# highfem/tqdne

Measured on AMD Instinct MI355X. Metric: waveforms/sec (train step + 18-step EDM sample), 3ch x 4096, higher is better.
Workload: dtype f32 (contractions on MFMA with fp32 accumulate: bf16x3, and fp16 + block-scaled-fp6 corrections on the 128/256-channel forward convs; sampler state f64)

## Files before the change

include/tqdne_hip.h:

```cpp
#ifndef TQDNE_HIP_H
#define TQDNE_HIP_H

#include <stddef.h>
#include <stdint.h>

#ifdef __cplusplus
extern "C" {
#endif

#ifndef __HIP__
typedef struct ihipStream_t* hipStream_t;
#endif

#define TQ_ABI_VERSION 8

#define TQ_ERR_ARG (-1)
#define TQ_ERR_SHAPE (-2)

#define TQ_CONV_GN 1
#define TQ_CONV_SILU 2
#define TQ_CONV_EMB 4
#define TQ_CONV_RES 8
#define TQ_CONV_STATS 16
#define TQ_CONV_DROPOUT 32
#define TQ_CONV_POLY2 64
#define TQ_CONV_CH_TILES 128
#define TQ_CONV_WIDE_TABLE 256

#define TQ_WFMT_BF16X3 0
#define TQ_WFMT_F16_MX8 1
#define TQ_WFMT_F16_MX6 2

typedef struct TqGnFold {
    const float* stats0;
    const float* stats1;
    int32_t slot0, slot1;
    const float* gamma;
    const float* beta;
    float* mean_rstd;
} TqGnFold;

typedef struct TqConvDesc {
    int32_t B, T_in, T_out;
    int32_t C_in0, C_in1;
    int32_t C_out;
    int32_t ktaps, stride, pad;
    int32_t upsample;
    int32_t flags;
    int32_t emb_stride;
    uint32_t dropout_site;
    float dropout_p;
    uint64_t dropout_seed;
    int32_t C_skip0, C_skip1;
    int32_t wfmt;
    int32_t* range_flag;
    const void* reserved1;
    int32_t t_tile;
    int32_t reserved2;
    const TqGnFold* gn_fold;
} TqConvDesc;

#define TQ_BWD_GN 1
#define TQ_BWD_SILU 2
#define TQ_BWD_DROPOUT 4
#define TQ_BWD_ACCUM 8
#define TQ_BWD_STATS 16

typedef struct TqConvBwdDesc {
    int32_t B, T;
    int32_t C_dy;
    int32_t C_dx0, C_dx1;
    int32_t ktaps;
    int32_t flags;
    uint32_t dropout_site;
    float dropout_p;
    uint64_t dropout_seed;
    int32_t wfmt;
    int32_t reserved;
    const uint32_t* dy_amax;
} TqConvBwdDesc;

int tq_abi_version(void);
int tq_build_flags(void);

size_t tq_conv_weight_pack_bytes(int C_out, int C_in, int K, int mode);
int tq_pack_conv_weight(const float* w, int C_out, int C_in, int K, int mode, void* packed, hipStream_t stream);
int tq_conv_tile_co(int C_out);
int tq_conv1d_max_cin(int wfmt, int C_out);
int tq_conv1d_max_cout(void);
size_t tq_conv1d_wide_lds_bytes(int ktaps, int t_tile, int C_out);
int tq_conv1d_gn_table_entries(int wide);
int tq_conv1d_gn_fold_max_cin(int wfmt, int t_tile, int C_out);
int tq_colsum_max_channels(void);
typedef struct TqPackJob {
    const void* src;
    void* dst;
    int32_t C_out, C_in, K, mode;
    int32_t block_begin;
    int32_t reserved;
} TqPackJob;
int tq_pack_job_blocks(int C_out, int C_in, int K, int mode);
int tq_pack_jobs(const TqPackJob* jobs_device, int njobs, int total_blocks, hipStream_t stream);

int tq_conv1d_fwd(const TqConvDesc* desc, const float* x0, const float* x1, const float* gscale, const float* gshift,
                  const void* packed_w, const float* bias, const float* emb, const float* residual, float* y,
                  float* stats_partial, hipStream_t stream);

int tq_conv1d_fwd_skip(const TqConvDesc* desc, const float* x0, const float* x1, const float* gscale, const float* gshift,
                       const void* packed_w_main_then_skip, const float* bias, const float* emb, const float* skip_x0,
                       const float* skip_x1, const float* skip_bias, float* y, float* stats_partial, hipStream_t stream);

#define TQ_KV_V_BF16 0
#define TQ_KV_V_F16 1
int tq_conv1d_fwd_qkv(const TqConvDesc* desc, const float* x, const float* gscale, const float* gshift, const void* packed_w,
                      const float* bias, float* qkv, void* kv_planes, int H, int D, int v_format, hipStream_t stream);

int tq_conv1d_bwd_data(const TqConvBwdDesc* desc, const float* dy, const void* packed_w_t, const float* x0, const float* x1,
                       const float* gscale, const float* gshift, float* dx0, float* dx1, float* gstats_partial,
                       hipStream_t stream);

size_t tq_conv1d_bwd_weight_workspace(const TqConvDesc* desc);
int tq_conv1d_bwd_weight(const TqConvDesc* desc, const float* dy, const float* x0, const float* x1, const float* gscale,
                         const float* gshift, float* dw, void* workspace, size_t ws_bytes, hipStream_t stream);
int tq_conv1d_bwd_weight_colsum(const TqConvDesc* desc, const float* dy, const float* x0, const float* x1, const float* gscale,
                                const float* gshift, float* dw, void* workspace, size_t ws_bytes, float* colsum_bc, int bc_stride,
                                float* colsum_c, float* colsum_c2, hipStream_t stream);

size_t tq_stem_conv_lds_bytes(int C_in, int C_out, int ktaps);
int tq_stem_conv_fwd(const float* x_nct, const float* in_scale, const float* w, const float* bias, float* y,
                     float* stats_partial, int B, int C_in, int T, int C_out, int ktaps, hipStream_t stream);

size_t tq_head_conv_lds_bytes(int C_in, int C_out, int ktaps);
int tq_head_conv_fwd(const float* x, const float* gscale, const float* gshift, const float* w, const float* bias,
                     const float* c_out, const float* c_skip, const float* skip_src, float* y_nct, int B, int T, int C_in,
                     int C_out, int ktaps, hipStream_t stream);

int tq_gn_finalize(const float* stats0, int C0, const float* stats1, int C1, int B, int T, const float* gamma,
                   const float* beta, float* gscale, float* gshift, float* mean_rstd, int slot0, int slot1, hipStream_t stream);

int tq_gn_bwd_finalize(const float* gstats_partial, const float* mean_rstd, const float* gamma, int B, int C, int T,
                       float* coef_a, float* coef_b, float* coef_c, float* dgamma, float* dbeta, hipStream_t stream);
int tq_gn_bwd_apply(const float* g, const float* x, const float* r, const float* coef_a, const float* coef_b,
                    const float* coef_c, float* dx, int B, int T, int C_src, int C_total, int c_offset, int accumulate,
                    hipStream_t stream);
int tq_gn_bwd_apply_colsum(const float* g, const float* x, const float* r, const float* coef_a, const float* coef_b,
                           const float* coef_c, float* dx, int B, int T, int C_src, int C_total, int c_offset, int accumulate,
                           float* colsum_bc, int bc_stride, float* colsum_c, float* colsum_c2, uint32_t* amax_out,
                           hipStream_t stream);
typedef struct TqGemmJob {
    const float* A;
    const float* B;
    float* C;
    const float* U;
    int32_t M, N, K;
    int32_t sam, sak, sbk, sbn, ldc, ldu;
    int32_t pre_b;
    int32_t tile_begin;
} TqGemmJob;
int tq_gemm_tiles(int M, int N);
int tq_gemm_f32_jobs(const TqGemmJob* jobs_device, int njobs, int total_tiles, hipStream_t stream);
int tq_fourier_features(const float* t, const float* W, float* out, int B, int half, hipStream_t stream);

#define TQ_AMAX_WAYS 16
#define TQ_AMAX_STRIDE 32
#define TQ_AMAX_WORDS (TQ_AMAX_WAYS * TQ_AMAX_STRIDE)
int tq_colsum(const float* dy, int B, int T, int C, float* out_bc, int bc_stride, float* out_c, float* out_c2,
              const float* bscale, uint32_t* amax_out, hipStream_t stream);
int tq_zero_stuff(const float* dy, float* out, int B, int T_out, int T_in, int C, hipStream_t stream);
int tq_pair_sum(const float* d_up, float* dx, int B, int T, int C, int accumulate, hipStream_t stream);
int tq_upsample_poly_wgrad_fold(const float* dw2, float* dw, int C_out, int C_in, hipStream_t stream);
int tq_stem_conv_bwd_weight(const float* dy, const float* x_nct, const float* in_scale, float* dw, int B, int C_in, int T,
                            int C_out, int ktaps, hipStream_t stream);
size_t tq_stem_head_bwd_workspace(void);
int tq_stem_conv_bwd_weight_ws(const float* dy, const float* x_nct, const float* in_scale, float* dw, int B, int C_in, int T,
                               int C_out, int ktaps, void* workspace, size_t ws_bytes, hipStream_t stream);
int tq_head_conv_bwd_ws(const float* dpred_nct, const float* c_out, const float* x, const float* gscale, const float* gshift,
                        const float* w, float* g_out, float* gstats_partial, float* dw, float* db, int B, int T, int C_in,
                        int C_out, int ktaps, void* workspace, size_t ws_bytes, hipStream_t stream);
size_t tq_head_conv_bwd_lds_bytes(int C_in, int C_out, int ktaps);
int tq_head_conv_bwd(const float* dpred_nct, const float* c_out, const float* x, const float* gscale, const float* gshift,
                     const float* w, float* g_out, float* gstats_partial, float* dw, float* db, int B, int T, int C_in,
                     int C_out, int ktaps, hipStream_t stream);

int tq_embed_fwd(const float* t, const float* cond, const float* fourier_w, const float* w0, const float* b0,
                 const float* w2, const float* b2, const float* cw0, const float* cb0, const float* cw2, const float* cb2,
                 float* emb, float* silu_emb, float* hidden ,
                 int B, int mc, int ncond, hipStream_t stream);

int tq_linear_fwd(const float* x, const float* w, const float* bias, float* out, int B, int E, int N, hipStream_t stream);

size_t tq_attention_workspace_bytes(int B, int T, int H, int D);
int tq_attention_fwd(const float* qkv, float* out, float* lse ,
                     void* workspace , int B, int T,
                     int H, int D, hipStream_t stream);
int tq_attention_fwd_presplit(const float* qkv, const void* kv_planes, float* out, int B, int T, int H, int D, int v_format,
                              hipStream_t stream);
int tq_attention_bwd(const float* qkv, const float* out, const float* dout, const float* lse, float* delta, float* dqkv, int B,
                     int T, int H, int D, hipStream_t stream);
int tq_attention_bwd_ws(const float* qkv, const float* out, const float* dout, const float* lse, float* delta, float* dqkv,
                        void* workspace, int B, int T, int H, int D, hipStream_t stream);
int tq_attention_bwd_ws_kv(const float* qkv, const float* out, const float* dout, const float* lse, float* delta, float* dqkv,
                           void* workspace, const void* kv_planes, int B, int T, int H, int D, hipStream_t stream);

int tq_attention_head_tile(int D);
size_t tq_attention_hd_lds_bytes(int D, int pass);
size_t tq_attention_hd_workspace_bytes(int B, int T, int H, int D);
int tq_attention_fwd_hd(const float* qkv, float* out, float* lse, void* workspace, int B, int T, int H, int D, hipStream_t stream);
int tq_attention_bwd_hd(const float* qkv, const float* out, const float* dout, const float* lse, float* delta, float* dqkv,
                        void* workspace, int B, int T, int H, int D, hipStream_t stream);

int tq_edm_scalars(const float* sigma, int sigma_stride, float sigma_data, float* c_in, float* c_out, float* c_skip,
                   float* c_noise, float* lweight, int B, hipStream_t stream);
int tq_cm_scalars(const float* sigma, int sigma_stride, float sigma_data, float sigma_min, float* c_out, float* c_skip,
                  int B, hipStream_t stream);
int tq_edm_noise_inject(const float* y, const float* unit_noise, const float* eps, float P_mean, float P_std,
                        float* sigma, float* x_noisy, int B, int n_per_sample, hipStream_t stream);
int tq_edm_loss(const float* pred, const float* y, const float* lweight, float* loss_out, float* dpred, int B,
                int n_per_sample, hipStream_t stream);
// ... 90 lines not shown
```

tqdne_amd/_lib.py:

```python

from __future__ import annotations

import ctypes as C
import os
from typing import Optional

from . import _build

_LIB = None

c_f32p = C.c_void_p
VP = C.c_void_p
I = C.c_int
F = C.c_float
SZ = C.c_size_t

TQ_CONV_GN, TQ_CONV_SILU, TQ_CONV_EMB, TQ_CONV_RES, TQ_CONV_STATS, TQ_CONV_DROPOUT = 1, 2, 4, 8, 16, 32
TQ_CONV_POLY2 = 64
TQ_CONV_CH_TILES = 128
TQ_CONV_WIDE_TABLE = 256
TQ_WFMT_BF16X3, TQ_WFMT_F16_MX8, TQ_WFMT_F16_MX6 = 0, 1, 2
TQ_KV_V_BF16, TQ_KV_V_F16 = 0, 1
PACK_MODE = {TQ_WFMT_BF16X3: 0, TQ_WFMT_F16_MX8: 2, TQ_WFMT_F16_MX6: 3}
PACK_MODE_T = {TQ_WFMT_BF16X3: 1, TQ_WFMT_F16_MX6: 5}


DEFAULT_SCHEME = "f16mx6"
ABI_VERSION = 8


def requested_scheme() -> str:
    v = os.environ.get("TQDNE_CONV_SCHEME", DEFAULT_SCHEME).lower()
    if v not in ("bf16x3", "f16mx8", "f16mx6"):
        raise ValueError(f"TQDNE_CONV_SCHEME={v!r}: expected bf16x3, f16mx8 or f16mx6")
    return v


def attn_v_format() -> int:
    if os.environ.get("TQDNE_ATTN_VF16", "1") == "0" or requested_scheme() == "bf16x3":
        return TQ_KV_V_BF16
    return TQ_KV_V_F16


MX6_C64 = os.environ.get("TQDNE_CONV_MX6_C64", "0") == "1"


WIDE_MX6 = os.environ.get("TQDNE_WIDE_MX6", "1") != "0"


def conv_max_cin(wfmt: int, C_out: int = 0) -> int:
    return load().tq_conv1d_max_cin(wfmt, C_out)


def forward_wfmt(C_out: int, sources, stride: int = 1, upsample: bool = False, k5_act: bool = False,
                 gn: Optional[bool] = None) -> int:
    v = requested_scheme()
    co_ok = C_out % 128 == 0 or (C_out % 64 == 0 and k5_act and not upsample and v == "f16mx6" and MX6_C64)
    ok = stride == 1 and co_ok and all(c % 64 == 0 for c in sources if c)
    if not ok or v == "bf16x3":
        return TQ_WFMT_BF16X3
    fmt = TQ_WFMT_F16_MX6 if v == "f16mx6" else TQ_WFMT_F16_MX8
    cin = sum(c for c in list(sources)[:2] if c)
    if gn is None or gn:
        if cin > conv_max_cin(fmt, C_out) or (cin > load().tq_conv1d_gn_table_entries(0) and not WIDE_MX6):
            return TQ_WFMT_BF16X3
    return fmt
TQ_BWD_GN, TQ_BWD_SILU, TQ_BWD_DROPOUT, TQ_BWD_ACCUM, TQ_BWD_STATS = 1, 2, 4, 8, 16
STAT_SLOT = 128
TQ_AMAX_WAYS, TQ_AMAX_STRIDE = 16, 32
TQ_AMAX_WORDS = TQ_AMAX_WAYS * TQ_AMAX_STRIDE


class TqGnFold(C.Structure):
    _fields_ = [("stats0", C.c_void_p), ("stats1", C.c_void_p), ("slot0", C.c_int32), ("slot1", C.c_int32),
                ("gamma", C.c_void_p), ("beta", C.c_void_p), ("mean_rstd", C.c_void_p)]


class TqConvDesc(C.Structure):
    _fields_ = [
        ("B", C.c_int32), ("T_in", C.c_int32), ("T_out", C.c_int32),
        ("C_in0", C.c_int32), ("C_in1", C.c_int32), ("C_out", C.c_int32),
        ("ktaps", C.c_int32), ("stride", C.c_int32), ("pad", C.c_int32),
        ("upsample", C.c_int32), ("flags", C.c_int32), ("emb_stride", C.c_int32),
        ("dropout_site", C.c_uint32), ("dropout_p", C.c_float), ("dropout_seed", C.c_uint64),
        ("C_skip0", C.c_int32), ("C_skip1", C.c_int32), ("wfmt", C.c_int32),
        ("range_flag", C.c_void_p), ("reserved1", C.c_void_p), ("t_tile", C.c_int32), ("reserved2", C.c_int32),
        ("gn_fold", C.POINTER(TqGnFold)),
    ]


class TqAdamChunk(C.Structure):
    _fields_ = [("p", C.c_void_p), ("g", C.c_void_p), ("m", C.c_void_p), ("v", C.c_void_p), ("ema", C.c_void_p),
                ("n", C.c_int32), ("reserved", C.c_int32)]


TQ_ADAM_CHUNK = 4096


class TqGemmJob(C.Structure):
    _fields_ = [("A", C.c_void_p), ("B", C.c_void_p), ("C", C.c_void_p), ("U", C.c_void_p),
                ("M", C.c_int32), ("N", C.c_int32), ("K", C.c_int32),
                ("sam", C.c_int32), ("sak", C.c_int32), ("sbk", C.c_int32), ("sbn", C.c_int32), ("ldc", C.c_int32), ("ldu", C.c_int32),
                ("pre_b", C.c_int32), ("tile_begin", C.c_int32)]


class TqPackJob(C.Structure):
    _fields_ = [("src", C.c_void_p), ("dst", C.c_void_p), ("C_out", C.c_int32), ("C_in", C.c_int32), ("K", C.c_int32),
                ("mode", C.c_int32), ("block_begin", C.c_int32), ("reserved", C.c_int32)]


class TqConvBwdDesc(C.Structure):
    _fields_ = [
        ("B", C.c_int32), ("T", C.c_int32), ("C_dy", C.c_int32), ("C_dx0", C.c_int32), ("C_dx1", C.c_int32),
        ("ktaps", C.c_int32), ("flags", C.c_int32), ("dropout_site", C.c_uint32), ("dropout_p", C.c_float),
        ("dropout_seed", C.c_uint64), ("wfmt", C.c_int32), ("reserved", C.c_int32), ("dy_amax", C.c_void_p),
    ]


_PROTOS = {
    "tq_abi_version": (I, []),
    "tq_build_flags": (I, []),
    "tq_conv_weight_pack_bytes": (SZ, [I, I, I, I]),
    "tq_pack_conv_weight": (I, [VP, I, I, I, I, VP, VP]),
    "tq_conv_tile_co": (I, [I]),
    "tq_conv1d_max_cin": (I, [I, I]),
    "tq_conv1d_max_cout": (I, []),
    "tq_conv1d_gn_table_entries": (I, [I]),
    "tq_conv1d_wide_lds_bytes": (SZ, [I, I, I]),
    "tq_conv1d_gn_fold_max_cin": (I, [I, I, I]),
    "tq_colsum_max_channels": (I, []),
    "tq_conv1d_fwd": (I, [C.POINTER(TqConvDesc)] + [VP] * 11),
    "tq_conv1d_fwd_skip": (I, [C.POINTER(TqConvDesc)] + [VP] * 13),
    "tq_stem_conv_fwd": (I, [VP] * 6 + [I] * 5 + [VP]),
    "tq_head_conv_fwd": (I, [VP] * 9 + [I] * 5 + [VP]),
    "tq_head_conv_lds_bytes": (SZ, [I, I, I]),
    "tq_stem_conv_lds_bytes": (SZ, [I, I, I]),
    "tq_head_conv_bwd_lds_bytes": (SZ, [I, I, I]),
    "tq_gn_finalize": (I, [VP, I, VP, I, I, I, VP, VP, VP, VP, VP, I, I, VP]),
    "tq_embed_fwd": (I, [VP] * 14 + [I, I, I, VP]),
    "tq_linear_fwd": (I, [VP] * 4 + [I, I, I, VP]),
    "tq_attention_fwd": (I, [VP, VP, VP, VP, I, I, I, I, VP]),
    "tq_attention_fwd_presplit": (I, [VP, VP, VP, I, I, I, I, I, VP]),
    "tq_conv1d_fwd_qkv": (I, [C.POINTER(TqConvDesc)] + [VP] * 7 + [I, I, I, VP]),
    "tq_attention_workspace_bytes": (SZ, [I, I, I, I]),
    "tq_attention_bwd": (I, [VP] * 6 + [I, I, I, I, VP]),
    "tq_attention_bwd_ws": (I, [VP] * 7 + [I, I, I, I, VP]),
    "tq_attention_bwd_ws_kv": (I, [VP] * 8 + [I, I, I, I, VP]),
    "tq_attention_head_tile": (I, [I]),
    "tq_attention_hd_lds_bytes": (SZ, [I, I]),
    "tq_attention_hd_workspace_bytes": (SZ, [I, I, I, I]),
    "tq_attention_fwd_hd": (I, [VP, VP, VP, VP, I, I, I, I, VP]),
    "tq_attention_bwd_hd": (I, [VP] * 7 + [I, I, I, I, VP]),
    "tq_edm_scalars": (I, [VP, I, F, VP, VP, VP, VP, VP, I, VP]),
    "tq_cm_scalars": (I, [VP, I, F, F, VP, VP, I, VP]),
    "tq_edm_noise_inject": (I, [VP, VP, VP, F, F, VP, VP, I, I, VP]),
    "tq_edm_loss": (I, [VP, VP, VP, VP, VP, I, I, VP]),
    "tq_heun_euler": (I, [VP] * 7 + [SZ, VP]),
    "tq_heun_correct": (I, [VP] * 8 + [SZ, VP]),
    "tq_sampler_init": (I, [VP] * 4 + [SZ, VP]),
    "tq_heun_churn": (I, [VP, VP, VP, C.c_double, VP, VP, SZ, VP]),
    "tq_axpy_sigma": (I, [VP, VP, VP, VP, I, I, VP]),
    "tq_pseudo_huber_loss": (I, [VP, VP, VP, F, VP, VP, I, I, VP]),
    "tq_mse_loss": (I, [VP, VP, VP, VP, SZ, VP]),
    "tq_scale_add2": (I, [VP, VP, VP, VP, VP, I, I, VP]),
    "tq_ddpm_step": (I, [VP, VP, VP, VP, SZ, I] + [C.c_double] * 6 + [VP]),
    "tq_vae_reparam_fwd": (I, [VP, VP, VP, VP, I, I, I, VP]),
    "tq_vae_reparam_bwd": (I, [VP, VP, VP, VP, F, I, I, I, VP]),
    "tq_concat_scale": (I, [VP, VP, VP, VP, I, I, I, I, VP]),
    "tq_envelope_fwd": (I, [VP, VP, I, I, I, I, C.c_double, C.c_double, VP]),
    "tq_envelope_inv": (I, [VP, VP, I, I, I, C.c_double, C.c_double, VP]),
    "tq_adam_ema_step": (I, [VP, I] + [C.c_double] * 8 + [VP]),
    "tq_adam_ema_step_guarded": (I, [VP, I] + [C.c_double] * 8 + [VP, VP]),
    "tq_radam_ema_step_guarded": (I, [VP, I] + [C.c_double] * 7 + [VP, VP]),
    "tq_adam_ema_step_clipped": (I, [VP, I] + [C.c_double] * 8 + [VP, VP, C.c_double, VP]),
    "tq_radam_ema_step_clipped": (I, [VP, I] + [C.c_double] * 7 + [VP, VP, C.c_double, VP]),
    "tq_grad_sumsq": (I, [VP, I, VP, VP]),
    "tq_grad_clip_coef": (I, [VP, I, C.c_double, C.c_double, VP, VP]),
    "tq_ema_swap": (I, [VP, I, VP]),
    "tq_conv1d_bwd_data": (I, [VP] * 11),
    "tq_conv1d_bwd_weight_workspace": (SZ, [VP]),
    "tq_conv1d_bwd_weight": (I, [VP] * 8 + [SZ, VP]),
    "tq_conv1d_bwd_weight_colsum": (I, [VP] * 8 + [SZ, VP, I, VP, VP, VP]),
    "tq_gn_bwd_finalize": (I, [VP, VP, VP, I, I, I, VP, VP, VP, VP, VP, VP]),
    "tq_gn_bwd_apply": (I, [VP] * 7 + [I] * 6 + [VP]),
    "tq_gn_bwd_apply_colsum": (I, [VP] * 7 + [I] * 6 + [VP, I, VP, VP, VP, VP]),
    "tq_pack_job_blocks": (I, [I, I, I, I]),
    "tq_pack_jobs": (I, [VP, I, I, VP]),
    "tq_gemm_tiles": (I, [I, I]),
    "tq_gemm_f32_jobs": (I, [VP, I, I, VP]),
    "tq_fourier_features": (I, [VP, VP, VP, I, I, VP]),
    "tq_colsum": (I, [VP, I, I, I, VP, I, VP, VP, VP, VP, VP]),
    "tq_zero_stuff": (I, [VP, VP, I, I, I, I, VP]),
    "tq_pair_sum": (I, [VP, VP, I, I, I, I, VP]),
    "tq_upsample_poly_wgrad_fold": (I, [VP, VP, I, I, VP]),
    "tq_stem_conv_bwd_weight": (I, [VP] * 4 + [I] * 5 + [VP]),
    "tq_head_conv_bwd": (I, [VP] * 10 + [I] * 5 + [VP]),
    "tq_stem_head_bwd_workspace": (SZ, []),
    "tq_stem_conv_bwd_weight_ws": (I, [VP] * 4 + [I] * 5 + [VP, SZ, VP]),
    "tq_head_conv_bwd_ws": (I, [VP] * 10 + [I] * 5 + [VP, SZ, VP]),
    "tq_boundary_max_channels": (I, []),
    "tq_nct_to_btc": (I, [VP] * 4 + [I] * 5 + [VP]),
    "tq_btc_to_nct": (I, [VP] * 5 + [I] * 5 + [VP]),
    "tq_avg_pool2_fwd": (I, [VP, VP, VP, I, I, I, VP]),
    "tq_nearest_up2_fwd": (I, [VP, VP, VP, I, I, I, VP]),
    "tq_avg_pool2_bwd": (I, [VP, VP, I, I, I, I, VP]),
    "tq_classifier_head_max_channels": (I, []),
    "tq_classifier_head_max_classes": (I, []),
    "tq_classifier_head_bwd_workspace": (SZ, [I, I]),
    "tq_classifier_head_fwd": (I, [VP] * 11 + [I] * 4 + [VP]),
    "tq_cross_entropy": (I, [VP, VP, VP, C.c_int64, VP, VP, I, I, VP]),
    "tq_classifier_head_bwd": (I, [VP] * 15 + [SZ] + [I] * 4 + [VP]),
}

def lib_path() -> str:
    return os.environ.get("TQDNE_HIP_LIB", _build.LIBPATH)


# ... 38 lines not shown
```

tqdne_amd/csrc/conv1d_fwd_wide.hip:

```cpp
#include "conv1d_kernel.hpp"

namespace {
template <int KT, int ACT, bool FUSE>
int dispatch_wide(const ConvArgs& a, hipStream_t s) {
    if (a.wfmt != TQ_WFMT_F16_MX6 || (a.flags & TQ_CONV_POLY2)) return TQ_ERR_SHAPE;
    if (a.C0 % 64 || a.C1 % 64 || a.sC0 % 64 || a.sC1 % 64 || a.C_out % 128) return TQ_ERR_SHAPE;
    if (a.t_tile == 32) {
        if constexpr (KT == 5 && ACT >= 2) return launch<KT, 1, 0, 4, 1, 0, ACT, FUSE, 2, false, 2, 2, CONV_GTAB_WIDE>(a, s);
        return TQ_ERR_SHAPE;
    }
    if (a.C_out % 256 == 0) return launch<KT, 1, 0, 8, 1, 0, ACT, FUSE, 2, false, 8, 2, CONV_GTAB_WIDE>(a, s);
    return launch<KT, 1, 0, 4, 1, 0, ACT, FUSE, 2, false, 8, 2, CONV_GTAB_WIDE>(a, s);
}
}

namespace tq {
int conv_launch_fwd_wide_k5(const ConvArgs& a, int act, bool fuse, hipStream_t s) {
    if (fuse) {
        if (act == 3) return dispatch_wide<5, 3, true>(a, s);
        if (act == 2) return dispatch_wide<5, 2, true>(a, s);
        return TQ_ERR_SHAPE;
    }
    if (act == 3) return dispatch_wide<5, 3, false>(a, s);
    if (act == 2) return dispatch_wide<5, 2, false>(a, s);
    if (act == 1) return dispatch_wide<5, 1, false>(a, s);
    return TQ_ERR_SHAPE;
}

int conv_launch_fwd_wide(const ConvArgs& a, int ktaps, int act, bool fuse, hipStream_t s) {
    if (ktaps == 5) return conv_launch_fwd_wide_k5(a, act, fuse, s);
    if (fuse) return TQ_ERR_SHAPE;
    return conv_launch_fwd_wide_k13(a, ktaps, act, s);
}
}

extern "C" int tq_conv1d_max_cin(int wfmt, int C_out) {
    if (C_out < 0 || C_out % 32) return 0;
    switch (wfmt) {
        case TQ_WFMT_F16_MX6:
            return (C_out % 128 == 0) ? CONV_GTAB_WIDE : (C_out % 64 == 0 ? CONV_GTAB_NARROW : 0);
        case TQ_WFMT_F16_MX8: return (C_out % 128 == 0) ? CONV_GTAB_NARROW : 0;
        case TQ_WFMT_BF16X3: return CONV_GTAB_WIDE;
        default: return 0;
    }
}

template <int KT>
static size_t wide_lds(int t_tile, int C_out) {
    if (C_out <= 0 || C_out % 128) return 0;
    if (t_tile == 32) return KT == 5 ? (size_t)ConvLds<KT, 1, 0, 4, 1, 0, 2, 2, false, 2, 2, CONV_GTAB_WIDE>::BYTES : 0;
    if (t_tile) return 0;
    return C_out % 256 == 0 ? (size_t)ConvLds<KT, 1, 0, 8, 1, 0, 2, 2, false, 8, 2, CONV_GTAB_WIDE>::BYTES
                            : (size_t)ConvLds<KT, 1, 0, 4, 1, 0, 2, 2, false, 8, 2, CONV_GTAB_WIDE>::BYTES;
}
extern "C" size_t tq_conv1d_wide_lds_bytes(int ktaps, int t_tile, int C_out) {
    return ktaps == 5 ? wide_lds<5>(t_tile, C_out) : ktaps == 3 ? wide_lds<3>(t_tile, C_out) : ktaps == 1 ? wide_lds<1>(t_tile, C_out) : 0;
}

extern "C" int tq_conv1d_gn_table_entries(int wide) { return wide ? CONV_GTAB_WIDE : CONV_GTAB_NARROW; }

extern "C" int tq_conv1d_max_cout(void) { return 3 * CONV_GTAB_NARROW; }

extern "C" int tq_conv1d_gn_fold_max_cin(int wfmt, int t_tile, int C_out) {
    if (C_out <= 0 || C_out % 32) return 0;
    int lim = 0;
    if (t_tile == 32) {
        if (wfmt == TQ_WFMT_F16_MX6) lim = C_out % 128 ? 0 : ConvLds<5, 1, 0, 4, 1, 0, 2, 2, false, 2, 2, 1024>::FOLD_MAX_CIN;
        else if (wfmt != TQ_WFMT_BF16X3) lim = 0;
        else if (C_out % 128 == 0) lim = ConvLds<5, 1, 0, 4, 1, 0, 2, 0, false, 2, 2, 1024>::FOLD_MAX_CIN;
        else if (C_out % 64 == 0) lim = ConvLds<5, 1, 0, 2, 1, 0, 2, 0, false, 2, 2, 1024>::FOLD_MAX_CIN;
        else lim = ConvLds<5, 1, 0, 1, 1, 0, 2, 0, false, 2, 2, 1024>::FOLD_MAX_CIN;
    } else if (t_tile == 0 && wfmt == TQ_WFMT_F16_MX6) {
        if (C_out % 256 == 0) lim = ConvLds<5, 1, 0, 8, 1, 0, 2, 2, false, 8, 2, 1024>::FOLD_MAX_CIN;
        else if (C_out % 128 == 0) lim = ConvLds<5, 1, 0, 4, 1, 0, 2, 2, false, 8, 2, 1024>::FOLD_MAX_CIN;
    }
    return lim / 32 * 32;
}
```

tqdne_amd/csrc/conv1d_kernel.hpp:

```cpp
#pragma once
#include <cmath>
#include <cstdlib>
#include <type_traits>

#include "common.hpp"
#include "conv_args.hpp"
#include "gn_fold.hpp"
#include <atomic>
#include "../../include/tqdne_hip.h"

using namespace tq;

#ifdef TQ_STAMP
static __device__ unsigned long long tq_stamps[12];
#ifdef TQ_STAMP_OWNER
extern "C" int tq_debug_read_stamps(unsigned long long* out, int reset) {
    hipError_t e = hipMemcpyFromSymbol(out, HIP_SYMBOL(tq_stamps), sizeof(unsigned long long) * 12);
    if (e != hipSuccess) return (int)e;
    if (reset) {
        unsigned long long z[12] = {0, 0, 0, 0, 0, 0, 0, 0, 0, 0, 0, 0};
        e = hipMemcpyToSymbol(HIP_SYMBOL(tq_stamps), z, sizeof(z));
    }
    return (int)e;
}
// ... 137 lines not shown
        const int coff = first ? cb : cb - c0;
        return src + (size_t)b * p.T_in * cs + coff + 4 * m;
    };

    auto load_one = [&](const float* base, int cs, int it) -> float4 __attribute__((always_inline)) {
        const int i = (tid + it * C::NTHR) / C::TPR;
        int pos = src_pos(i);
        pos = pos < 0 ? 0 : (pos >= T_src ? T_src - 1 : pos);
        const int srow = UPS ? (pos >> 1) : pos;
        return *reinterpret_cast<const float4*>(base + (size_t)srow * cs);
    };

    auto write_one = [&](int chunk, int buf, int it, const float4& rv) __attribute__((always_inline)) {
        unsigned char* hi_plane = lds + buf * C::BUF;
        unsigned char* lo_plane = hi_plane + C::PLANE;
        const int i = (tid + it * C::NTHR) / C::TPR;
        const int pos = src_pos(i);
        const float msk = (pos >= 0 && pos < T_src) ? 1.f : 0.f;
        float u[4] = {rv.x, rv.y, rv.z, rv.w};
        const bool act = !(FUSE && chunk >= nchunks);
        if (ACT >= 1 && act) {
            u[0] = fmaf(g_a.x, u[0], g_s.x); u[1] = fmaf(g_a.y, u[1], g_s.y);
            u[2] = fmaf(g_a.z, u[2], g_s.z); u[3] = fmaf(g_a.w, u[3], g_s.w);
        }
        if (ACT >= 2 && act) {
#pragma unroll
            for (int j = 0; j < 4; ++j)
                u[j] = u[j] * __builtin_amdgcn_rcpf(1.0f + __builtin_amdgcn_exp2f(u[j] * -1.4426950408889634f));
        }
        if (ACT == 3 && act) {
            const int cb = chunk * C::CH;
            const int pc = pos < 0 ? 0 : pos;
            const uint32_t e0 = (uint32_t)pc * (uint32_t)Cin + (uint32_t)(cb + 4 * m);
#pragma unroll
            for (int j = 0; j < 4; ++j)
                u[j] = (drop_hash(dkey, e0 + j) >= p.drop_thresh) ? u[j] * p.drop_scale : 0.f;
        }
        if constexpr (SCH == 0) {
            uint32_t hb[4];
            float lo[4];
#pragma unroll
            for (int j = 0; j < 4; ++j) {
                u[j] *= msk;
                hb[j] = __float_as_uint(u[j]) & 0xFFFF0000u;
                lo[j] = u[j] - __uint_as_float(hb[j]);
            }
            uint2 hv;
            hv.x = (hb[0] >> 16) | hb[1];
            hv.y = (hb[2] >> 16) | hb[3];
            bf16x4 l;
            l[0] = (__bf16)lo[0]; l[1] = (__bf16)lo[1]; l[2] = (__bf16)lo[2]; l[3] = (__bf16)lo[3];
            const int off = i * 64 + ((wslot ^ (((i >> 2) & 1) << 1)) << 4) + (whalf << 3);
            *reinterpret_cast<uint2*>(hi_plane + off) = hv;
            *reinterpret_cast<bf16x4*>(lo_plane + off) = l;
        } else {
            f16x4 hv;
            float xl[4], xc[4];
#pragma unroll
            for (int j = 0; j < 4; ++j) {
                u[j] *= msk;
                hv[j] = (_Float16)u[j];
                xl[j] = __builtin_amdgcn_fmed3f(u[j] - (float)hv[j], -0.109375f, 0.109375f);
                xc[j] = __builtin_amdgcn_fmed3f(u[j], -448.f, 448.f);
            }
            i16x2 c8 = {0, 0};
            c8 = __builtin_amdgcn_cvt_scalef32_pk_fp8_f32(c8, xl[0], xl[1], 0.000244140625f, false);
            c8 = __builtin_amdgcn_cvt_scalef32_pk_fp8_f32(c8, xl[2], xl[3], 0.000244140625f, true);
            int x8 = __builtin_amdgcn_cvt_pk_fp8_f32(xc[0], xc[1], 0, false);
            x8 = __builtin_amdgcn_cvt_pk_fp8_f32(xc[2], xc[3], x8, true);
            const int sw = i & 7;
            const int row = i * 128;
            *reinterpret_cast<f16x4*>(hi_plane + row + ((wslot ^ sw) << 4) + (whalf << 3)) = hv;
            const int g = m >> 2, byte = (m & 3) << 2;
            *reinterpret_cast<i16x2*>(lo_plane + row + ((g ^ sw) << 4) + byte) = c8;
            *reinterpret_cast<int*>(lo_plane + row + (((4 + g) ^ sw) << 4) + byte) = x8;
        }
    };

    const int m2 = tid & 3;
    float4 raw2[4];
    float nlog2e = -1.4426950408889634f, n4096 = -4096.f;
    asm volatile("" : "+s"(nlog2e), "+s"(n4096));

    float* gtab = reinterpret_cast<float*>(lds + (PW ? 4 * C::BUF : C::LDS_BYTES));
    constexpr bool FOLD_LATE0 = SCH == 0 && TBW == 2 && ACT >= 1 && !PW && EPI == 0;
    const bool fold0_pending = FOLD_LATE0 && p.cf_st0 != nullptr;
    auto chunk_base2 = [&](int stage, int& cs) -> const float* __attribute__((always_inline)) {
        const bool sk = FUSE && stage >= nchunks;
        const int cb = (sk ? stage - nchunks : stage) * C::CH;
        const float* a0 = sk ? p.sx0 : p.x0;
        const float* a1 = sk ? p.sx1 : p.x1;
        const int c0 = sk ? p.sC0 : p.C0, c1 = sk ? p.sC1 : p.C1;
        const bool first = cb < c0;
        cs = first ? c0 : c1;
        return (first ? a0 : a1) + (size_t)b * p.T_in * cs + (first ? cb : cb - c0) + 16 * m2;
    };
    auto load16 = [&](const float* base, int cs, int row, float4 (&v)[4]) __attribute__((always_inline)) {
        int pos = src_pos(row);
        pos = pos < 0 ? 0 : (pos >= T_src ? T_src - 1 : pos);
        const float4* q = reinterpret_cast<const float4*>(base + (size_t)(UPS ? (pos >> 1) : pos) * cs);
        v[0] = q[0]; v[1] = q[1]; v[2] = q[2]; v[3] = q[3];
    };
    auto write16 = [&](int chunk, int buf, int row, const float4 (&v)[4]) __attribute__((always_inline)) {
        unsigned char* hi_plane = lds + buf * C::BUF;
        unsigned char* lo_plane = hi_plane + C::PLANE;
        const int pos = src_pos(row);
        const float msk = (pos >= 0 && pos < T_src) ? 1.f : 0.f;
        float u[16] = {v[0].x, v[0].y, v[0].z, v[0].w, v[1].x, v[1].y, v[1].z, v[1].w,
                       v[2].x, v[2].y, v[2].z, v[2].w, v[3].x, v[3].y, v[3].z, v[3].w};
        const bool act = !(FUSE && chunk >= nchunks);
        if (ACT >= 1 && act) {
            const int cb = chunk * C::CH + 16 * m2;
            const float4* ga = reinterpret_cast<const float4*>(gtab + cb);
            const float4* gs = reinterpret_cast<const float4*>(gtab + Cin + cb);
#pragma unroll
            for (int q4 = 0; q4 < 4; ++q4) {
                const float4 a = ga[q4], sh = gs[q4];
                u[4 * q4 + 0] = fmaf(a.x, u[4 * q4 + 0], sh.x); u[4 * q4 + 1] = fmaf(a.y, u[4 * q4 + 1], sh.y);
                u[4 * q4 + 2] = fmaf(a.z, u[4 * q4 + 2], sh.z); u[4 * q4 + 3] = fmaf(a.w, u[4 * q4 + 3], sh.w);
            }
        }
        if (ACT >= 2 && act) {
            const float one = (pos >= 0 && pos < T_src) ? 1.0f : __builtin_inff();
#pragma unroll
            for (int j = 0; j < 16; j += 2) {
                f32x2 uu = {u[j], u[j + 1]};
                f32x2 e = uu * nlog2e;
                e = f32x2{__builtin_amdgcn_exp2f(e.x), __builtin_amdgcn_exp2f(e.y)} + one;
                uu = uu * f32x2{__builtin_amdgcn_rcpf(e.x), __builtin_amdgcn_rcpf(e.y)};
                u[j] = uu.x; u[j + 1] = uu.y;
            }
        }
        const float mm = (ACT >= 2 && act) ? 1.f : msk * dy_scale;
        if (ACT == 3 && act) {
            const int pc = pos < 0 ? 0 : pos;
            const uint32_t e0 = (uint32_t)pc * (uint32_t)Cin + (uint32_t)(chunk * C::CH + 16 * m2);
            unsigned keep = 0;
#pragma unroll 4
            for (int j = 0; j < 16; ++j)
                keep |= (drop_hash(dkey, e0 + j) >= p.drop_thresh ? 1u : 0u) << j;
#pragma unroll
            for (int j = 0; j < 16; ++j) u[j] = ((keep >> j) & 1u) ? u[j] * p.drop_scale : 0.f;
        }
        f16x8 h0, h1;
        f32x16 xl, xf;
        float mx = 0.f;
#pragma unroll
        for (int j = 0; j < 16; j += 2) {
            f32x2 x = {u[j], u[j + 1]};
            if constexpr (ACT < 2 || FUSE) x = x * mm;
            typedef _Float16 f16x2 __attribute__((ext_vector_type(2)));
            const f16x2 hp = {(_Float16)x.x, (_Float16)x.y};
            if (j < 8) { h0[j] = hp.x; h0[j + 1] = hp.y; } else { h1[j - 8] = hp.x; h1[j - 7] = hp.y; }
            const f32x2 x4k = x * 4096.f;
            float r0, r1;
            const unsigned hpu = __builtin_bit_cast(unsigned, hp);
            asm("v_fma_mix_f32 %0, %1, %2, %3 op_sel_hi:[1,0,0]" : "=v"(r0) : "v"(hpu), "s"(n4096), "v"(x4k.x));
            asm("v_fma_mix_f32 %0, %1, %2, %3 op_sel:[1,0,0] op_sel_hi:[1,0,0]" : "=v"(r1) : "v"(hpu), "s"(n4096), "v"(x4k.y));
            xl[j] = r0; xl[j + 1] = r1; xf[j] = x.x; xf[j + 1] = x.y;
            mx = fmaxf(fmaxf(mx, fabsf(r0)), fabsf(x.x));
            mx = fmaxf(fmaxf(mx, fabsf(r1)), fabsf(x.y));
        }
        const unsigned bb = e8m0_block_scale(mx);
        const u32x6 pk = cvt_2xpk16_fp6(xl, xf, __uint_as_float(bb << 23));
        const int sw = row & 7;
        const int ro = row * 128;
        *reinterpret_cast<uint4*>(hi_plane + ro + (((2 * m2) ^ sw) << 4)) = __builtin_bit_cast(uint4, h0);
        *reinterpret_cast<uint4*>(hi_plane + ro + (((2 * m2 + 1) ^ sw) << 4)) = __builtin_bit_cast(uint4, h1);
// ... 180 lines not shown
#pragma unroll
            for (int cbk = 0; cbk < 2; ++cbk)
                acc[cbk][tb] = __builtin_amdgcn_mfma_f32_16x16x32_f16(__builtin_bit_cast(f16x8, w[cbk * 4 + 1].u), b1v, acc[cbk][tb], 0, 0, 0);
#pragma unroll
            for (int cbk = 0; cbk < 2; ++cbk) {
                const Frag& c0 = w[cbk * 4 + 2];
                const Frag& c1 = w[cbk * 4 + 3];
                const i32x8 ac = {(int)c0.u.x, (int)c0.u.y, (int)c0.u.z, (int)c0.u.w, (int)c1.u.x, (int)c1.u.y, (int)c1.u.z, (int)c1.u.w};
#ifdef TQ_ABL_FP6TIME
                acc[cbk][tb] = __builtin_amdgcn_mfma_scale_f32_16x16x128_f8f6f4(ac, bc, acc[cbk][tb], 2, 2, 0, 127, 0, 115);
#else
                acc[cbk][tb] = __builtin_amdgcn_mfma_scale_f32_16x16x128_f8f6f4(ac, bc, acc[cbk][tb], 0, 0, 0, 127, 0, 115);
#endif
            }
        }
    };

#ifndef TQ_LDS_DEPTH
#define TQ_LDS_DEPTH 2
#endif
#ifndef TQ_LDS_DEPTH1
#define TQ_LDS_DEPTH1 1
#endif
    Frag wa[C::NW], wb[C::NW];
#ifndef TQ_LDS_DEPTH2
#define TQ_LDS_DEPTH2 1
#endif
    constexpr int LDS_DEP = SCH == 2 ? TQ_LDS_DEPTH2 : (SCH ? TQ_LDS_DEPTH1 : TQ_LDS_DEPTH);

    auto mma_stream = [&](const unsigned char* hi_plane, const unsigned char* lo_plane, int s0, auto ntaps_c, auto first_tap_c)
        __attribute__((always_inline)) {
        constexpr int NTAPS = decltype(ntaps_c)::value, K0 = decltype(first_tap_c)::value;
        constexpr int DEP = LDS_DEP, NB = LDS_DEP + 1, NS = NTAPS * TBW;
        Frag bf[NB][C::NBF];
        int b0 = tap_base(K0), b0n = b0;
#pragma unroll
        for (int t = 0; t < DEP; ++t) read_b(hi_plane, lo_plane, b0, t, bf[t]);
#pragma unroll
        for (int st = 0; st < NS; ++st) {
            const int kk = st / TBW, tb = st % TBW;
            if (tb == 0 && kk + 1 < NTAPS) b0n = tap_base(K0 + kk + 1);
            const int sn = st + DEP;
            if (sn < NS) read_b(hi_plane, lo_plane, (sn / TBW) == kk ? b0 : b0n, sn % TBW, bf[sn % NB]);
            __builtin_amdgcn_sched_barrier(0);
            if (kk & 1) mma_step(wb, bf[st % NB], tb); else mma_step(wa, bf[st % NB], tb);
            __builtin_amdgcn_sched_barrier(0);
            if (tb == TBW - 1) {
                const int nxt = (NTAPS == 1) ? (s0 + 1) : ((kk + 2 < NTAPS) ? (s0 + kk + 2) : ((kk & 1) ? (s0 + NTAPS + 1) : (s0 + NTAPS)));
                if (kk & 1) load_w(nxt, wb); else load_w(nxt, wa);
                b0 = b0n;
                __builtin_amdgcn_sched_barrier(0);
            }
        }
    };

    auto compute = [&](int chunk, int buf) __attribute__((always_inline)) {
        const unsigned char* hi_plane = lds + buf * C::BUF;
        mma_stream(hi_plane, hi_plane + C::PLANE, chunk * KT, std::integral_constant<int, KT>{}, std::integral_constant<int, 0>{});
    };

    auto compute_skip = [&](int j, int buf) __attribute__((always_inline)) {
        const unsigned char* hi_plane = lds + buf * C::BUF;
        const unsigned char* lo_plane = hi_plane + C::PLANE;
        constexpr int DEP = LDS_DEP, NB = LDS_DEP + 1;
        Frag bf[NB][C::NBF];
        const int b0 = tap_base(C::PAD);
#pragma unroll
        for (int t = 0; t < DEP; ++t) read_b(hi_plane, lo_plane, b0, t, bf[t]);
#pragma unroll
        for (int tb = 0; tb < TBW; ++tb) {
            if (tb + DEP < TBW) read_b(hi_plane, lo_plane, b0, tb + DEP, bf[(tb + DEP) % NB]);
            __builtin_amdgcn_sched_barrier(0);
            mma_step(wa, bf[tb % NB], tb);
            __builtin_amdgcn_sched_barrier(0);
        }
#pragma unroll
        for (int q = 0; q < C::NW; ++q) wa[q] = wb[q];
        load_w(nchunks * KT + j + 2, wb);
        __builtin_amdgcn_sched_barrier(0);
    };

    static_assert(!(SCH == 2 && ACT >= 1) || C::NTHR >= 256, "one table entry per thread");
    constexpr int GT_N = GTW / 1024;
    constexpr bool FOLD_LATE = SCH == 2 && ACT >= 1 && !PW && EPI == 0 && (TBW == 8 || TBW == 2);
    const bool fold_late = FOLD_LATE && p.cf_st0 != nullptr;
    float4 gt_a = make_float4(0.f, 0.f, 0.f, 0.f), gt_s = gt_a;
    int gt_i = 0;
    if constexpr (SCH == 2 && ACT >= 1) {
        const int n4 = Cin >> 2;
        gt_i = tid < n4 ? tid : n4 - 1;
        if (!fold_late) {
            gt_a = reinterpret_cast<const float4*>(p.gscale + (size_t)b * Cin)[gt_i];
            gt_s = reinterpret_cast<const float4*>(p.gshift + (size_t)b * Cin)[gt_i];
        }
    }
    float4 gt_a2 = make_float4(0.f, 0.f, 0.f, 0.f), gt_s2 = gt_a2;
    int gt_i2 = 0;
    if constexpr (SCH == 2 && ACT >= 1 && GT_N == 2) {
        static_assert(GT_N == 1 || 2 * C::NTHR * 4 >= GTW, "two table entries per thread cover the wide table");
        const int n4 = Cin >> 2;
        gt_i2 = tid + C::NTHR < n4 ? tid + C::NTHR : n4 - 1;
        gt_a2 = reinterpret_cast<const float4*>(p.gscale + (size_t)b * Cin)[gt_i2];
        gt_s2 = reinterpret_cast<const float4*>(p.gshift + (size_t)b * Cin)[gt_i2];
    }
    auto gtab_store = [&]() __attribute__((always_inline)) {
        if constexpr (SCH == 2 && ACT >= 1) {
            if constexpr (FOLD_LATE) {
                if (fold_late) {
                    gn_fold_sample<false, false>(reinterpret_cast<double*>(lds), b, p.cf_st0, p.C0, p.cf_st1, p.C1, p.T_in, p.cf_ns0, p.cf_ns1,
                                                 p.cf_gamma, p.cf_beta, const_cast<float*>(p.gscale), const_cast<float*>(p.gshift), p.cf_mean_rstd,
                                                 gtab, gtab + Cin);
                    __syncthreads();
                    return;
                }
            }
            float4* g4 = reinterpret_cast<float4*>(gtab);
            g4[gt_i] = gt_a;
            g4[(Cin >> 2) + gt_i] = gt_s;
            if constexpr (GT_N == 2) {
                g4[gt_i2] = gt_a2;
                g4[(Cin >> 2) + gt_i2] = gt_s2;
            }
            __syncthreads();
        }
    };
    if constexpr (PW) gtab_store();
    const int npass = PW ? n_ctiles : 1;
    if constexpr (PW) {
        static_assert(!PW || SCH == 2 || C::NIT == C::PRE, "PW stages a chunk in PRE iterations");
        static_assert(!PW || SCH != 2 || (C::NFULL == 1 && C::HALO_TASKS == 0), "PW, scheme 2: one 16-channel task per thread and chunk");
        if constexpr (SCH == 2) {
            float4 rr2[4][4];
#pragma unroll
            for (int c = 0; c < 4; ++c) {
                int cs2;
                const float* base2 = chunk_base2(c < nchunks ? c : nchunks - 1, cs2);
                load16(base2, cs2, tid >> 2, rr2[c]);
            }
            load_w(0, wa);
            load_w(1, wb);
#pragma unroll
            for (int c = 0; c < 4; ++c) write16(c < nchunks ? c : nchunks - 1, c, tid >> 2, rr2[c]);
            __syncthreads();
        } else {
        float4 rr[4][C::PRE], ga4[4], gs4[4];
#pragma unroll
        for (int c = 0; c < 4; ++c) {
            const int cc = c < nchunks ? c : nchunks - 1;
            int cs;
            const float* base = chunk_base(cc, cs);
#pragma unroll
            for (int it = 0; it < C::PRE; ++it) rr[c][it] = load_one(base, cs, it);
            if (ACT >= 1) {
                ga4[c] = *reinterpret_cast<const float4*>(p.gscale + (size_t)b * Cin + cc * C::CH + 4 * m);
                gs4[c] = *reinterpret_cast<const float4*>(p.gshift + (size_t)b * Cin + cc * C::CH + 4 * m);
            }
        }
        load_w(0, wa);
        load_w(1, wb);
#pragma unroll
        for (int c = 0; c < 4; ++c) {
            if (ACT >= 1) { g_a = ga4[c]; g_s = gs4[c]; }
#pragma unroll
            for (int it = 0; it < C::PRE; ++it) write_one(c < nchunks ? c : nchunks - 1, c, it, rr[c][it]);
        }
        __syncthreads();
        }
    }
    int pass = 0;
next_pass:
    if constexpr (PW) {
#pragma unroll
        for (int i = 0; i < 2; ++i)
#pragma unroll
            for (int j = 0; j < 8; ++j) acc[i][j] = f32x4{0.f, 0.f, 0.f, 0.f};
        for (int j = 0; 2 * j < nchunks; ++j) {
            pw_c0 = 2 * j;
            mma_stream(lds, lds + C::PLANE, 2 * j, std::integral_constant<int, 2>{}, std::integral_constant<int, 0>{});
        }
        if (pass + 1 < npass) wbase += (size_t)(C::MT >> 4) * C::NWB * 64;
        load_w(0, wa);
        load_w(1, wb);
        __builtin_amdgcn_sched_barrier(0);
    } else {
        stage_load(0);
        if (wave_active) {
            load_w(0, wa);
            if (KT > 1 || nskip > 0) load_w(1, wb);
        }
        gtab_store();
        if constexpr (FOLD_LATE0) {
            if (fold0_pending) {
                gn_fold_sample<false, false>(reinterpret_cast<double*>(lds), b, p.cf_st0, p.C0, p.cf_st1, p.C1, p.T_in, p.cf_ns0, p.cf_ns1, p.cf_gamma,
                                             p.cf_beta, const_cast<float*>(p.gscale), const_cast<float*>(p.gshift), p.cf_mean_rstd, gtab, gtab + Cin);
                __syncthreads();
                g_a = *reinterpret_cast<const float4*>(gtab + 4 * m);
                g_s = *reinterpret_cast<const float4*>(gtab + Cin + 4 * m);
            }
        }
        stage_write(0, 0);
        __syncthreads();
#ifdef TQ_STAMP
        unsigned long long s_load = 0, s_mma = 0, s_write = 0, s_bar = 0;
        const unsigned long long t_begin = __builtin_amdgcn_s_memtime();
        if (tid == 0 && blockIdx.x < 4096) {
            unsigned long long* tl = tq_timeline + blockIdx.x * 8;
            tl[0] = r_entry; tl[1] = __builtin_amdgcn_s_memrealtime(); tl[4] = t_entry; tl[5] = t_begin;
        }
#endif
        if constexpr (!FUSE) {
            for (int c = 0; c + 1 < nstages; ++c) {
                TQ_T(tA)
#ifndef TQ_ABL_NOSTAGE
                stage_load(c + 1);
#endif
                TQ_T(tB)
                if (wave_active) {
                    if (!FUSE || c < nchunks) compute(c, c & 1);
                    else compute_skip(c - nchunks, c & 1);
                }
                TQ_T(tC)
#ifndef TQ_ABL_NOSTAGE
                stage_write(c + 1, (c + 1) & 1);
// ... 281 lines not shown
#pragma unroll
                        for (int j = 0; j < 4; ++j) v[j] *= dsilu_f(a4[j] * xv[j] + h4[j]);
                    }
                    if (p.bflags & TQ_BWD_DROPOUT) {
                        const uint32_t e0 = (uint32_t)t * (uint32_t)Ctot + (uint32_t)co;
#pragma unroll
                        for (int j = 0; j < 4; ++j)
                            v[j] = (drop_hash(dkey, e0 + j) >= p.drop_thresh) ? v[j] * p.drop_scale : 0.f;
                    }
                    if (accum) {
                        f32x4 r = lq[tb][cbk];
                        if (need_x) r = *reinterpret_cast<const f32x4*>(dst[cbk] + o);
                        v[0] += r[0]; v[1] += r[1]; v[2] += r[2]; v[3] += r[3];
                    }
                    *reinterpret_cast<float4*>(dst[cbk] + o) = make_float4(v[0], v[1], v[2], v[3]);
#pragma unroll
                    for (int j = 0; j < 4; ++j) { s1[cbk][j] += v[j]; s2[cbk][j] += v[j] * xv[j]; }
                }
            }
        }
        if (p.bflags & TQ_BWD_STATS) {
#pragma unroll
            for (int cbk = 0; cbk < 2; ++cbk) {
                const int co = co_wave + cbk * 16 + 4 * (lane >> 4);
#pragma unroll
                for (int j = 0; j < 4; ++j) {
#pragma unroll
                    for (int o = 1; o < 16; o <<= 1) {
                        s1[cbk][j] += __shfl_xor(s1[cbk][j], o);
                        s2[cbk][j] += __shfl_xor(s2[cbk][j], o);
                    }
                }
                if constexpr (TBW == 8) {
                    if ((lane & 15) == 0 && slot < p.nslots) {
                        float* st = p.stats + (((size_t)b * p.nslots + slot) * Ctot + co) * 2;
                        *reinterpret_cast<float4*>(st) = make_float4(s1[cbk][0], s2[cbk][0], s1[cbk][1], s2[cbk][1]);
                        *reinterpret_cast<float4*>(st + 4) = make_float4(s1[cbk][2], s2[cbk][2], s1[cbk][3], s2[cbk][3]);
                    }
                }
            }
            if constexpr (TBW == 4) {
                __syncthreads();
                float* red = reinterpret_cast<float*>(lds) + (wm * 4 + (lane >> 4)) * 16;
                if (wn == 1 && (lane & 15) == 0) {
#pragma unroll
                    for (int cbk = 0; cbk < 2; ++cbk)
#pragma unroll
                        for (int j = 0; j < 4; ++j) { red[(cbk * 4 + j) * 2] = s1[cbk][j]; red[(cbk * 4 + j) * 2 + 1] = s2[cbk][j]; }
                }
                __syncthreads();
                if (wn == 0 && (lane & 15) == 0 && slot < p.nslots) {
#pragma unroll
                    for (int cbk = 0; cbk < 2; ++cbk) {
                        const int co = co_wave + cbk * 16 + 4 * (lane >> 4);
                        float a1[4], a2[4];
#pragma unroll
                        for (int j = 0; j < 4; ++j) { a1[j] = s1[cbk][j] + red[(cbk * 4 + j) * 2]; a2[j] = s2[cbk][j] + red[(cbk * 4 + j) * 2 + 1]; }
                        float* st = p.stats + (((size_t)b * p.nslots + slot) * Ctot + co) * 2;
                        *reinterpret_cast<float4*>(st) = make_float4(a1[0], a2[0], a1[1], a2[1]);
                        *reinterpret_cast<float4*>(st + 4) = make_float4(a1[2], a2[2], a1[3], a2[3]);
                    }
                }
            }
        }
    }
    if constexpr (PW) {
        co_wave += C::MT;
        if (++pass < npass) goto next_pass;
    }
#ifdef TQ_STAMP
    if (tid == 0 && blockIdx.x < 4096) {
        unsigned long long* tl = tq_timeline + blockIdx.x * 8;
        tl[3] = __builtin_amdgcn_s_memrealtime(); tl[7] = __builtin_amdgcn_s_memtime();
    }
#endif
}

template <int KT, int STRIDE, int UPS, int WM, int WN, int EPI, int ACT, int SCH, bool PW, int TBW, int NCB, int GTW>
struct ConvLds {
    using C = Cfg<KT, STRIDE, UPS, WM, WN, SCH, TBW, NCB>;
    static constexpr int GTAB_MAX = ((SCH == 2 && ACT >= 1) || (SCH == 0 && TBW == 2 && ACT >= 1 && !PW && EPI == 0)) ? 2 * 4 * GTW : 0;
    static constexpr int STAGE = PW ? 4 * C::BUF : C::LDS_BYTES;
    static constexpr int BYTES = STAGE + GTAB_MAX;
    static constexpr int FOLD_MAX_CIN = GTW != 1024 ? 0 : ((STAGE / 8 - 64) / 2 < 1024 ? (STAGE / 8 - 64) / 2 : 1024);
};
constexpr int TQ_LDS_WORKGROUP_MAX = 163840;

template <int KT, int STRIDE, int UPS, int WM, int WN, int EPI, int ACT, bool FUSE, int SCH = 0, bool PW = false, int TBW = 8, int NCB = 2, int GTW = 1024>
int launch(const ConvArgs& a, hipStream_t stream) {
    using C = Cfg<KT, STRIDE, UPS, WM, WN, SCH, TBW, NCB>;
    using L = ConvLds<KT, STRIDE, UPS, WM, WN, EPI, ACT, SCH, PW, TBW, NCB, GTW>;
    auto kern = conv1d_mfma_kernel<KT, STRIDE, UPS, WM, WN, EPI, ACT, FUSE, SCH, PW, TBW, NCB, GTW>;
    constexpr int GTAB_MAX = L::GTAB_MAX;
    constexpr int LDS_BYTES = L::BYTES;
    static_assert(LDS_BYTES <= TQ_LDS_WORKGROUP_MAX, "tile + coefficient table exceed the LDS a workgroup may declare");
    if (a.cf_st0 && GTW != 1024) return TQ_ERR_SHAPE;
    if (GTAB_MAX && a.cf_st0 && a.C0 + a.C1 > 1024) return TQ_ERR_SHAPE;
    if (SCH == 2 && ACT >= 1 && a.C0 + a.C1 > GTW) return TQ_ERR_SHAPE;
    if (a.cf_st0) {
        constexpr bool built = (TBW == 2 && ACT >= 1 && !PW && EPI == 0) || (SCH == 2 && ACT >= 1 && !PW && EPI == 0 && TBW == 8);
        if (!built || (size_t)(2 * (a.C0 + a.C1) + 64) * sizeof(double) > (size_t)(LDS_BYTES - GTAB_MAX)) return TQ_ERR_SHAPE;
    }
    static std::atomic<uint64_t> attr_done{0};
    int dev_ord = 0;
    (void)hipGetDevice(&dev_ord);
    const uint64_t dev_bit = 1ull << (dev_ord & 63);
    if (!(attr_done.load(std::memory_order_acquire) & dev_bit)) {
        hipError_t e = hipFuncSetAttribute(reinterpret_cast<const void*>(kern),
                                           hipFuncAttributeMaxDynamicSharedMemorySize, LDS_BYTES);
        if (e != hipSuccess) return (int)e;
        attr_done.fetch_or(dev_bit, std::memory_order_release);
    }
    const int n_ttiles = (a.T_out + C::NT - 1) / C::NT;
    const int n_ctiles = (a.C_out + C::MT - 1) / C::MT;
    const unsigned grid = (unsigned)(a.B * n_ttiles * (PW ? 1 : n_ctiles));
    hipLaunchKernelGGL(kern, dim3(grid), dim3(C::NTHR), LDS_BYTES, stream, a);
    TQ_CHECK_LAUNCH();
    return 0;
}

template <int KT, int STRIDE, int UPS, int EPI, int ACT, bool FUSE = false>
int dispatch_tile(const ConvArgs& a, hipStream_t s) {
    if (a.t_tile == 32) {
        if constexpr (KT == 5 && STRIDE == 1 && UPS == 0 && EPI == 0 && ACT >= 2) {
            if (a.flags & TQ_CONV_POLY2) return TQ_ERR_SHAPE;
            if (a.wfmt == TQ_WFMT_F16_MX6) {
                if (a.C0 % 64 || a.C1 % 64 || a.sC0 % 64 || a.sC1 % 64 || a.C_out % 128) return TQ_ERR_SHAPE;
                if (conv_wide_table(a)) return conv_launch_fwd_wide(a, KT, ACT, FUSE, s);
                return launch<KT, STRIDE, UPS, 4, 1, EPI, ACT, FUSE, 2, false, 2>(a, s);
            }
            if (a.wfmt != TQ_WFMT_BF16X3) return TQ_ERR_SHAPE;
            if (a.C_out % 128 == 0) return launch<KT, STRIDE, UPS, 4, 1, EPI, ACT, FUSE, 0, false, 2>(a, s);
            if (a.C_out % 64 == 0) return launch<KT, STRIDE, UPS, 2, 1, EPI, ACT, FUSE, 0, false, 2>(a, s);
            return launch<KT, STRIDE, UPS, 1, 1, EPI, ACT, FUSE, 0, false, 2>(a, s);
        }
        return TQ_ERR_SHAPE;
    }
    if (a.wfmt == TQ_WFMT_F16_MX6) {
        if constexpr (STRIDE == 1 && UPS == 0 && EPI == 1 && ACT == 0 && !FUSE) {
            if (a.C0 % 64 || a.C1) return TQ_ERR_SHAPE;
            if (a.C_out % 256 == 0) return launch<KT, STRIDE, UPS, 8, 1, EPI, ACT, FUSE, 2>(a, s);
            if (a.C_out % 128 == 0) return launch<KT, STRIDE, UPS, 4, 1, EPI, ACT, FUSE, 2>(a, s);
            if (a.C_out % 64 == 0) return launch<KT, STRIDE, UPS, 2, 2, EPI, ACT, FUSE, 2, false, 4>(a, s);
            return TQ_ERR_SHAPE;
        }
        if constexpr (STRIDE == 1 && EPI != 1) {
            if (a.C0 % 64 || a.C1 % 64 || a.sC0 % 64 || a.sC1 % 64) return TQ_ERR_SHAPE;
            if constexpr (UPS == 0 && EPI == 0 && ACT >= 1) {
                if (conv_wide_table(a)) return conv_launch_fwd_wide(a, KT, ACT, FUSE, s);
            }
            if constexpr (KT == 1 && UPS == 0 && ACT <= 1) {
                const int cin = a.C0 + a.C1;
                const bool pw = !(a.flags & TQ_CONV_CH_TILES);
                if (pw && a.C_out % 256 == 0 && a.C_out >= 512 && (cin == 128 || cin == 256))
                    return launch<KT, STRIDE, UPS, 8, 1, EPI, ACT, FUSE, 2, true>(a, s);
            }
            if (a.C_out % 256 == 0) return launch<KT, STRIDE, UPS, 8, 1, EPI, ACT, FUSE, 2>(a, s);
            if (a.C_out % 128 == 0) return launch<KT, STRIDE, UPS, 4, 1, EPI, ACT, FUSE, 2>(a, s);
            if constexpr (KT == 5 && UPS == 0 && EPI == 0 && ACT >= 2) {
                if (a.C_out % 64 == 0 && !(a.flags & TQ_CONV_POLY2)) return launch<KT, STRIDE, UPS, 2, 2, EPI, ACT, FUSE, 2, false, 4>(a, s);
            }
        }
        return TQ_ERR_SHAPE;
    }
    if (a.wfmt == TQ_WFMT_F16_MX8) {
        if constexpr (STRIDE == 1 && EPI != 1) {

            if (a.C0 % 64 || a.C1 % 64 || a.sC0 % 64 || a.sC1 % 64) return TQ_ERR_SHAPE;
            if constexpr (KT == 1 && UPS == 0 && ACT <= 1) {
                const int cin = a.C0 + a.C1;
                if (a.C_out % 256 == 0 && a.C_out >= 512 && (cin == 128 || cin == 256))
                    return launch<KT, STRIDE, UPS, 8, 1, EPI, ACT, FUSE, 1, true>(a, s);
            }
            if (a.C_out % 256 == 0) return launch<KT, STRIDE, UPS, 8, 1, EPI, ACT, FUSE, 1>(a, s);
            if (a.C_out % 128 == 0) return launch<KT, STRIDE, UPS, 4, 1, EPI, ACT, FUSE, 1>(a, s);
        }
        return TQ_ERR_SHAPE;
    }
    if (a.wfmt != TQ_WFMT_BF16X3) return TQ_ERR_ARG;
    if constexpr (STRIDE == 1 && UPS == 0) {
        if (a.C_out % 256 == 0) return launch<KT, STRIDE, UPS, 8, 1, EPI, ACT, FUSE>(a, s);
    }
    if (a.C_out % 128 == 0) return launch<KT, STRIDE, UPS, 4, 1, EPI, ACT, FUSE>(a, s);
    if constexpr (STRIDE == 1) {
// ... 27 lines not shown
```

tqdne_amd/csrc/conv1d_mfma.hip:

```cpp
#include <cmath>

#include "common.hpp"
#include "conv_args.hpp"
#include "../../include/tqdne_hip.h"

using namespace tq;

extern "C" int tq_conv_tile_co(int C_out) {
    if (C_out % 128 == 0) return 128;
    if (C_out % 64 == 0) return 64;
    return 32;
}

static int conv1d_fwd_impl(const TqConvDesc* d, const float* x0, const float* x1, const float* gscale, const float* gshift,
                           const void* wpk, const float* bias, const float* emb, const float* res, const float* skip_x0,
                           const float* skip_x1, const float* skip_bias, float* y, float* stats, hipStream_t stream,
                           unsigned char* kv_planes = nullptr, int kvH = 0, int kvD = 0, int kvTp = 0, float kvscale = 1.f, int kv_vf16 = 0);

extern "C" int tq_conv1d_fwd_qkv(const TqConvDesc* d, const float* x, const float* gscale, const float* gshift, const void* wpk,
                                 const float* bias, float* qkv, void* kv_planes, int H, int D, int v_format, hipStream_t stream) {
    if (!d || !kv_planes || H <= 0 || (D != 32 && D != 64)) return TQ_ERR_ARG;
    if (v_format != TQ_KV_V_BF16 && v_format != TQ_KV_V_F16) return TQ_ERR_ARG;
    if (d->ktaps != 1 || d->stride != 1 || d->upsample || d->C_in1 || d->C_out != 3 * H * D || (d->C_skip0 | d->C_skip1)) return TQ_ERR_SHAPE;
    if (d->flags & (TQ_CONV_EMB | TQ_CONV_RES | TQ_CONV_STATS | TQ_CONV_DROPOUT | TQ_CONV_SILU)) return TQ_ERR_ARG;
    const int Tp = (d->T_out + 63) / 64 * 64;
    const float scale = (float)(1.0 / sqrt(sqrt((double)D)));
    return conv1d_fwd_impl(d, x, nullptr, gscale, gshift, wpk, bias, nullptr, nullptr, nullptr, nullptr, nullptr, qkv, nullptr, stream,
                           reinterpret_cast<unsigned char*>(kv_planes), H, D, Tp, scale, v_format == TQ_KV_V_F16 ? 1 : 0);
}

extern "C" int tq_conv1d_fwd(const TqConvDesc* d, const float* x0, const float* x1, const float* gscale,
                             const float* gshift, const void* wpk, const float* bias, const float* emb,
                             const float* res, float* y, float* stats, hipStream_t stream) {
    if (d && (d->C_skip0 || d->C_skip1)) return TQ_ERR_ARG;
    return conv1d_fwd_impl(d, x0, x1, gscale, gshift, wpk, bias, emb, res, nullptr, nullptr, nullptr, y, stats, stream);
}

extern "C" int tq_conv1d_fwd_skip(const TqConvDesc* d, const float* x0, const float* x1, const float* gscale,
                                  const float* gshift, const void* wpk_main_then_skip, const float* bias, const float* emb,
                                  const float* skip_x0, const float* skip_x1, const float* skip_bias, float* y, float* stats,
                                  hipStream_t stream) {
    if (!d || !skip_x0 || d->C_skip0 <= 0 || d->C_skip0 % 32 || d->C_skip1 < 0 || d->C_skip1 % 32) return TQ_ERR_ARG;
    if (d->C_skip1 > 0 && !skip_x1) return TQ_ERR_ARG;
    if (d->stride != 1 || d->upsample || (d->flags & TQ_CONV_RES)) return TQ_ERR_SHAPE;
    return conv1d_fwd_impl(d, x0, x1, gscale, gshift, wpk_main_then_skip, bias, emb, nullptr, skip_x0, skip_x1, skip_bias, y,
                           stats, stream);
}

static int conv1d_fwd_impl(const TqConvDesc* d, const float* x0, const float* x1, const float* gscale, const float* gshift,
                           const void* wpk, const float* bias, const float* emb, const float* res, const float* skip_x0,
                           const float* skip_x1, const float* skip_bias, float* y, float* stats, hipStream_t stream,
                           unsigned char* kv_planes, int kvH, int kvD, int kvTp, float kvscale, int kv_vf16) {
    if (!d || !x0 || !wpk || !y) return TQ_ERR_ARG;
    if (d->C_in0 <= 0 || d->C_in0 % 32 || d->C_in1 < 0 || d->C_in1 % 32 || d->C_out <= 0 || d->C_out % 32) return TQ_ERR_SHAPE;
    if (d->C_in1 > 0 && !x1) return TQ_ERR_ARG;
    if ((d->flags & TQ_CONV_GN) && (!gscale || !gshift)) return TQ_ERR_ARG;
    if ((d->flags & TQ_CONV_EMB) && !emb) return TQ_ERR_ARG;
    if ((d->flags & TQ_CONV_RES) && !res) return TQ_ERR_ARG;
    if ((d->flags & TQ_CONV_STATS) && !stats) return TQ_ERR_ARG;
    if (d->B <= 0 || d->T_in <= 0 || d->T_out <= 0) return TQ_ERR_SHAPE;
    if (d->stride == 1) {
        const int Tsrc = d->upsample ? 2 * d->T_in : d->T_in;
        if (d->T_out != Tsrc || d->pad != d->ktaps / 2) return TQ_ERR_SHAPE;
    } else if (d->stride == 2) {
        if (d->ktaps != 3 || d->pad != 1 || d->upsample || d->T_out != (d->T_in + 2 - 3) / 2 + 1) return TQ_ERR_SHAPE;
    } else {
        return TQ_ERR_SHAPE;
    }
    ConvArgs a;
    a.x0 = x0; a.x1 = x1; a.gscale = gscale; a.gshift = gshift;
    a.wpk = reinterpret_cast<const uint4*>(wpk);
    a.bias = bias; a.emb = emb; a.res = res; a.y = y; a.stats = stats;
    a.B = d->B; a.T_in = d->T_in; a.T_out = d->T_out; a.C0 = d->C_in0; a.C1 = d->C_in1; a.C_out = d->C_out;
    a.emb_stride = d->emb_stride; a.flags = d->flags;
    const int tile = tq_conv_tile_co(d->C_out);
    a.ncob_pad = ((d->C_out + tile - 1) / tile) * tile / 16;
    a.nslots = (d->T_out + STAT_SLOT - 1) / STAT_SLOT;
    a.t_tile = 0;
    if (d->t_tile) {
        const int need = TQ_CONV_GN | TQ_CONV_SILU;
        if (d->t_tile != 32) return TQ_ERR_ARG;
        if (d->ktaps != 5 || d->stride != 1 || d->upsample || kv_planes || (d->flags & need) != need || (d->flags & TQ_CONV_POLY2))
            return TQ_ERR_SHAPE;
        a.t_tile = 32;
        a.nslots = (d->T_out + 31) / 32;
    }
    if (d->flags & TQ_CONV_POLY2) {
        if (d->ktaps != 3 || d->stride != 1 || d->upsample || (d->C_out & 63) || kv_planes || d->C_skip0 || d->C_skip1) return TQ_ERR_SHAPE;
        if ((d->flags & TQ_CONV_STATS) && d->T_out % STAT_SLOT && d->T_out % STAT_SLOT <= STAT_SLOT / 2) return TQ_ERR_SHAPE;
        a.nslots *= 2;
    }
    a.drop_site = d->dropout_site;
    a.drop_seed = d->dropout_seed;
    float pdrop = d->dropout_p;
    if (!(d->flags & TQ_CONV_DROPOUT) || pdrop <= 0.f) { a.flags &= ~TQ_CONV_DROPOUT; pdrop = 0.f; }
    if (pdrop >= 1.f) return TQ_ERR_ARG;
    a.drop_thresh = (uint32_t)((double)pdrop * 4294967296.0);
    a.drop_scale = 1.0f / (1.0f - pdrop);
    a.fx0 = a.fx1 = a.fgs = a.fgh = nullptr; a.y1 = nullptr; a.OC0 = d->C_out; a.bflags = 0;
    a.sx0 = skip_x0; a.sx1 = skip_x1; a.sbias = skip_bias; a.sC0 = d->C_skip0; a.sC1 = d->C_skip1;
    a.wfmt = d->wfmt;
    a.kv = kv_planes; a.kvH = kvH; a.kvD = kvD; a.kvTp = kvTp; a.kvscale = kvscale; a.kv_vf16 = (kv_planes && kv_vf16) ? 1 : 0;
    a.range_flag = d->range_flag;
    a.in_amax = nullptr;
    a.cf_st0 = a.cf_st1 = a.cf_gamma = a.cf_beta = nullptr; a.cf_mean_rstd = nullptr; a.cf_ns0 = a.cf_ns1 = 0;
    if (d->gn_fold) {
        const TqGnFold* f = d->gn_fold;
        if (!(d->flags & TQ_CONV_GN) || kv_planes || (a.t_tile != 32 && d->wfmt != TQ_WFMT_F16_MX6)) return TQ_ERR_SHAPE;
        if (!f->stats0 || !f->gamma || !f->beta || (d->C_in1 > 0 && !f->stats1)) return TQ_ERR_ARG;
        const int s0 = f->slot0 ? f->slot0 : STAT_SLOT, s1 = f->slot1 ? f->slot1 : STAT_SLOT;
        if ((s0 != STAT_SLOT && s0 != 32) || (s1 != STAT_SLOT && s1 != 32)) return TQ_ERR_ARG;
        if ((d->C_in0 + d->C_in1) % GN_GROUPS) return TQ_ERR_SHAPE;
        a.cf_st0 = f->stats0; a.cf_st1 = d->C_in1 > 0 ? f->stats1 : nullptr;
        a.cf_ns0 = (d->T_in + s0 - 1) / s0; a.cf_ns1 = (d->T_in + s1 - 1) / s1;
        a.cf_gamma = f->gamma; a.cf_beta = f->beta; a.cf_mean_rstd = f->mean_rstd;
    }
    if (d->reserved1) return TQ_ERR_ARG;

    if (d->stride == 2 || d->upsample) {
        if (a.flags & (TQ_CONV_GN | TQ_CONV_SILU | TQ_CONV_DROPOUT)) return TQ_ERR_SHAPE;
        return conv_launch_resample(a, d->ktaps, d->stride, stream);
    }
    if (a.kv) {
        return conv_launch_qkv(a, stream);
    }
    switch (d->ktaps) {
        case 1: return conv_launch_fwd_k1(a, stream);
        case 3: return conv_launch_fwd_k3(a, stream);
        case 5: return conv_launch_fwd_k5(a, stream);
        default: return TQ_ERR_SHAPE;
    }
}

extern "C" int tq_conv1d_bwd_data(const TqConvBwdDesc* d, const float* dy, const void* wpk_t, const float* x0,
                                  const float* x1, const float* gscale, const float* gshift, float* dx0, float* dx1,
                                  float* gstats, hipStream_t stream) {
    if (!d || !dy || !wpk_t || !dx0) return TQ_ERR_ARG;
    if (d->C_dy <= 0 || d->C_dy % 32 || d->C_dx0 <= 0 || d->C_dx0 % 32 || d->C_dx1 < 0 || d->C_dx1 % 32) return TQ_ERR_SHAPE;
    if (d->C_dx1 > 0 && !dx1) return TQ_ERR_ARG;
    const int need_x = d->flags & (TQ_BWD_GN | TQ_BWD_SILU | TQ_BWD_STATS);
    if (need_x && (!x0 || (d->C_dx1 > 0 && !x1))) return TQ_ERR_ARG;
    if ((d->flags & TQ_BWD_GN) && (!gscale || !gshift)) return TQ_ERR_ARG;
    if ((d->flags & TQ_BWD_STATS) && !gstats) return TQ_ERR_ARG;
    if (d->B <= 0 || d->T <= 0 || (d->ktaps != 1 && d->ktaps != 3 && d->ktaps != 5)) return TQ_ERR_SHAPE;
    ConvArgs a;
    a.x0 = dy; a.x1 = nullptr; a.gscale = nullptr; a.gshift = nullptr;
    a.wpk = reinterpret_cast<const uint4*>(wpk_t);
    a.bias = nullptr; a.emb = nullptr; a.res = nullptr; a.y = dx0; a.stats = gstats;
    a.B = d->B; a.T_in = d->T; a.T_out = d->T; a.C0 = d->C_dy; a.C1 = 0; a.C_out = d->C_dx0 + d->C_dx1;
    a.emb_stride = 0; a.flags = 0;
    const int tile = tq_conv_tile_co(a.C_out);
    a.ncob_pad = ((a.C_out + tile - 1) / tile) * tile / 16;
    a.nslots = (d->T + STAT_SLOT - 1) / STAT_SLOT;
    a.drop_site = d->dropout_site; a.drop_seed = d->dropout_seed;
    float pdrop = d->dropout_p;
    a.bflags = d->flags;
    if (!(d->flags & TQ_BWD_DROPOUT) || pdrop <= 0.f) { a.bflags &= ~TQ_BWD_DROPOUT; pdrop = 0.f; }
    if (pdrop >= 1.f) return TQ_ERR_ARG;
    a.drop_thresh = (uint32_t)((double)pdrop * 4294967296.0);
    a.drop_scale = 1.0f / (1.0f - pdrop);
    a.fx0 = x0; a.fx1 = x1; a.fgs = gscale; a.fgh = gshift; a.y1 = dx1; a.OC0 = d->C_dx0;
    a.sx0 = a.sx1 = a.sbias = nullptr; a.sC0 = a.sC1 = 0;
    a.wfmt = TQ_WFMT_BF16X3;
    a.in_amax = nullptr;
    a.t_tile = 0;
    if (d->wfmt == TQ_WFMT_F16_MX6) {
        if (!d->dy_amax) return TQ_ERR_ARG;
        if (d->C_dy % 64 || a.C_out % 64) return TQ_ERR_SHAPE;
        a.wfmt = TQ_WFMT_F16_MX6;
        a.in_amax = d->dy_amax;
    } else if (d->wfmt != TQ_WFMT_BF16X3) {
        return TQ_ERR_ARG;
    }
    a.kv = nullptr; a.kvH = a.kvD = a.kvTp = 0; a.kvscale = 1.f; a.kv_vf16 = 0;
    a.range_flag = nullptr;
    a.cf_st0 = a.cf_st1 = a.cf_gamma = a.cf_beta = nullptr; a.cf_mean_rstd = nullptr; a.cf_ns0 = a.cf_ns1 = 0;
    return conv_launch_dgrad(a, d->ktaps, stream);
}

namespace {
__device__ __forceinline__ void pack_mx_body(const float* __restrict__ w, int C_out, int C_in, int K, int ncob_pad,
                                             uint4* __restrict__ out, size_t gid) {
    const int nchunks = (C_in + 63) / 64;
    const size_t total = (size_t)nchunks * K * ncob_pad * 64;
    if (gid >= total) return;
    const int lane = gid & 63;
    size_t r = gid >> 6;
    const int cob = r % ncob_pad; r /= ncob_pad;
    const int tap = r % K;
    const int chunk = r / K;
    const int row = cob * 16 + (lane & 15), kq = lane >> 4;
// ... 202 lines not shown
```

tqdne_amd/csrc/conv_args.hpp:

```cpp
#pragma once
#include "common.hpp"
#include "../../include/tqdne_hip.h"

namespace tq {

struct ConvArgs {
    const float* x0;
    const float* x1;
    const float* gscale;
    const float* gshift;
    const uint4* wpk;
    const float* bias;
    const float* emb;
    const float* res;
    float* y;
    float* stats;
    int B, T_in, T_out, C0, C1, C_out;
    int emb_stride, flags, ncob_pad, nslots;
    uint32_t drop_site;
    uint32_t drop_thresh;
    float drop_scale;
    uint64_t drop_seed;
    const float* fx0;
    const float* fx1;
    const float* fgs;
    const float* fgh;
    float* y1;
    int OC0;
    int bflags;
    const float* sx0;
    const float* sx1;
    const float* sbias;
    int sC0, sC1;
    int wfmt;
    unsigned char* kv;
    int kvH, kvD, kvTp;
    float kvscale;
    int kv_vf16;
    int* range_flag;
    int t_tile;
    const uint32_t* in_amax;
    const float* cf_st0;
    const float* cf_st1;
    int cf_ns0, cf_ns1;
    const float* cf_gamma;
    const float* cf_beta;
    float* cf_mean_rstd;
};


typedef float f32x16 __attribute__((ext_vector_type(16)));
typedef float f32x2 __attribute__((ext_vector_type(2)));
typedef unsigned u32x6 __attribute__((ext_vector_type(6)));

__device__ __forceinline__ u32x6 cvt_2xpk16_fp6(const f32x16& a, const f32x16& b, float scale) {
    u32x6 out;
    asm volatile("v_cvt_scalef32_2xpk16_fp6_f32 %0, %1, %2, %3" : "=&v"(out) : "v"(a), "v"(b), "v"(scale));
    return out;
}
__device__ __forceinline__ unsigned e8m0_block_scale(float mx) {
    const unsigned b = (__float_as_uint(mx * (1.0f / 7.5f)) + 0x7FFFFFu) >> 23;
    return b < 13u ? 13u : (b > 254u ? 254u : b);
}


int conv_launch_fwd_k1(const ConvArgs& a, hipStream_t stream);
int conv_launch_fwd_k3(const ConvArgs& a, hipStream_t stream);
int conv_launch_fwd_k5(const ConvArgs& a, hipStream_t stream);
int conv_launch_fwd_k5b(const ConvArgs& a, hipStream_t stream);
int conv_launch_qkv(const ConvArgs& a, hipStream_t stream);
int conv_launch_resample(const ConvArgs& a, int ktaps, int stride, hipStream_t stream);
int conv_launch_dgrad(const ConvArgs& a, int ktaps, hipStream_t stream);
constexpr int CONV_GTAB_NARROW = 1024, CONV_GTAB_WIDE = 2048;
inline bool conv_wide_table(const ConvArgs& a) { return a.C0 + a.C1 > CONV_GTAB_NARROW || (a.flags & TQ_CONV_WIDE_TABLE); }
int conv_launch_fwd_wide(const ConvArgs& a, int ktaps, int act, bool fuse, hipStream_t stream);
int conv_launch_fwd_wide_k5(const ConvArgs& a, int act, bool fuse, hipStream_t stream);
int conv_launch_fwd_wide_k13(const ConvArgs& a, int ktaps, int act, hipStream_t stream);

}
```

tqdne_amd/csrc/small_ops.hip:

```cpp
#include "common.hpp"
#include "gn_fold.hpp"
#include "ends_wide.hpp"
#include "../../include/tqdne_hip.h"

using namespace tq;

extern "C" int tq_abi_version(void) { return TQ_ABI_VERSION; }
extern "C" int tq_build_flags(void) { return 0; }

namespace {
__global__ __launch_bounds__(256) void gn_finalize_kernel(const float* __restrict__ st0, int C0,
                                                          const float* __restrict__ st1, int C1, int T, int nslots0, int nslots1,
                                                          const float* __restrict__ gamma, const float* __restrict__ beta,
                                                          float* __restrict__ gscale, float* __restrict__ gshift,
                                                          float* __restrict__ mean_rstd) {
    extern __shared__ double sh[];
    gn_fold_sample<false, false>(sh, blockIdx.x, st0, C0, st1, C1, T, nslots0, nslots1, gamma, beta, gscale, gshift, mean_rstd);
}
}

extern "C" int tq_gn_finalize(const float* stats0, int C0, const float* stats1, int C1, int B, int T, const float* gamma,
                              const float* beta, float* gscale, float* gshift, float* mean_rstd, int slot0, int slot1,
                              hipStream_t stream) {
    if (!stats0 || !gamma || !beta || !gscale || !gshift || (C1 > 0 && !stats1)) return TQ_ERR_ARG;
// ... 53 lines not shown
            const int ii = i < nkc ? i : 0;
            wr[i] = *reinterpret_cast<const float4*>(ws + ii * C_out + 4 * cg);
            if (i >= nkc) wr[i] = make_float4(0.f, 0.f, 0.f, 0.f);
            const int k = ii / C_in, ci = ii % C_in;
            xoff[i] = ci * TW + k;
        }
        for (int tl = tr; tl < STAT_SLOT; tl += nrow) {
            const int t = t0 + tl;
            if (t >= T) break;
            float4 a = bv;
#pragma unroll
            for (int i = 0; i < 16; ++i) {
                if (i < nkc) {
                    const float xv = xs[xoff[i] + tl];
                    a.x = fmaf(wr[i].x, xv, a.x); a.y = fmaf(wr[i].y, xv, a.y);
                    a.z = fmaf(wr[i].z, xv, a.z); a.w = fmaf(wr[i].w, xv, a.w);
                }
            }
            *reinterpret_cast<float4*>(y + ((size_t)b * T + t) * C_out + 4 * cg) = a;
            s1[0] += a.x; s1[1] += a.y; s1[2] += a.z; s1[3] += a.w;
            s2[0] += a.x * a.x; s2[1] += a.y * a.y; s2[2] += a.z * a.z; s2[3] += a.w * a.w;
        }
    } else if (tr < nrow) {
        for (int tl = tr; tl < STAT_SLOT; tl += nrow) {
            const int t = t0 + tl;
            if (t >= T) break;
            float4 a = bv;
            for (int k = 0; k < KT; ++k)
                for (int ci = 0; ci < C_in; ++ci) {
                    const float xv = xs[ci * TW + tl + k];
                    const float4 wv = *reinterpret_cast<const float4*>(ws + (k * C_in + ci) * C_out + 4 * cg);
                    a.x = fmaf(wv.x, xv, a.x); a.y = fmaf(wv.y, xv, a.y);
                    a.z = fmaf(wv.z, xv, a.z); a.w = fmaf(wv.w, xv, a.w);
                }
            *reinterpret_cast<float4*>(y + ((size_t)b * T + t) * C_out + 4 * cg) = a;
            s1[0] += a.x; s1[1] += a.y; s1[2] += a.z; s1[3] += a.w;
            s2[0] += a.x * a.x; s2[1] += a.y * a.y; s2[2] += a.z * a.z; s2[3] += a.w * a.w;
        }
    }
    if (stats) {
        if (tr < nrow) {
#pragma unroll
            for (int j = 0; j < 4; ++j) {
                red[(tr * C_out + 4 * cg + j) * 2] = s1[j];
                red[(tr * C_out + 4 * cg + j) * 2 + 1] = s2[j];
            }
        }
        __syncthreads();
        for (int c = threadIdx.x; c < C_out; c += 256) {
            float a1 = 0.f, a2 = 0.f;
            for (int r = 0; r < nrow; ++r) { a1 += red[(r * C_out + c) * 2]; a2 += red[(r * C_out + c) * 2 + 1]; }
            float* st = stats + (((size_t)b * nslots + slot) * C_out + c) * 2;
            st[0] = a1; st[1] = a2;
        }
    }
}
}

extern "C" int tq_stem_conv_fwd(const float* x, const float* in_scale, const float* w, const float* bias, float* y,
                                float* stats, int B, int C_in, int T, int C_out, int ktaps, hipStream_t stream) {
    if (!x || !w || !y) return TQ_ERR_ARG;
    if (B <= 0 || T <= 0 || C_in <= 0 || C_in > 16 || C_out < 4 || C_out % 4 || C_out > 1024 || 256 % (C_out / 4))
        return ends_wide_stem_fwd(x, in_scale, w, bias, y, stats, B, C_in, T, C_out, ktaps, stream);
    const int nslots = (T + STAT_SLOT - 1) / STAT_SLOT;
    const int ngrp = C_out / 4, nrow = 256 / ngrp;
    const size_t sh = ((size_t)C_in * (STAT_SLOT + ktaps - 1) + (size_t)ktaps * C_in * C_out + (size_t)nrow * C_out * 2) * sizeof(float);
    if (sh > 160 * 1024) return ends_wide_stem_fwd(x, in_scale, w, bias, y, stats, B, C_in, T, C_out, ktaps, stream);
#define TQ_STEM(K)                                                                                          \
    {                                                                                                       \
        auto kern = stem_conv_kernel<K>;                                                                    \
        if (sh > 64 * 1024) (void)hipFuncSetAttribute(reinterpret_cast<const void*>(kern), hipFuncAttributeMaxDynamicSharedMemorySize, (int)sh); \
        hipLaunchKernelGGL(kern, dim3(B * nslots), dim3(256), sh, stream, x, in_scale, w, bias, y, stats, C_in, T, C_out, nslots); \
    }
    if (ktaps == 5) TQ_STEM(5)
    else if (ktaps == 3) TQ_STEM(3)
    else if (ktaps == 1) TQ_STEM(1)
    else return TQ_ERR_SHAPE;
#undef TQ_STEM
    TQ_CHECK_LAUNCH();
    return 0;
}

namespace {
template <int KT, int MAXCO>
__global__ __launch_bounds__(256) void head_conv_kernel(const float* __restrict__ x, const float* __restrict__ gscale,
                                                        const float* __restrict__ gshift, const float* __restrict__ w,
                                                        const float* __restrict__ bias, const float* __restrict__ c_out,
                                                        const float* __restrict__ c_skip, const float* __restrict__ skip_src,
                                                        float* __restrict__ y, int T, int C_in, int C_out, int ntiles) {
    extern __shared__ __attribute__((aligned(16))) float shm[];
    constexpr int PAD = KT / 2;
    constexpr int TW = 128;
    constexpr int NOUT = TW - (KT - 1);
    constexpr int NP = KT * MAXCO;
    constexpr int MAXV = 8;
    float* wl = shm;
    float* part = wl + C_in * NP;
    for (int i = threadIdx.x; i < C_in * NP; i += 256) {
        const int co = i % MAXCO, r = i / MAXCO;
        const int k = r % KT, ci = r / KT;
        wl[i] = (co < C_out) ? w[((size_t)co * C_in + ci) * KT + k] : 0.f;
    }
    const int tile = blockIdx.x % ntiles;
    const int b = blockIdx.x / ntiles;
    const int t0 = tile * NOUT;
    const int q = threadIdx.x & 3;
    const int nv = C_in >> 4;
    float4 ga[MAXV], gs[MAXV];
#pragma unroll
    for (int jv = 0; jv < MAXV; ++jv) {
        ga[jv] = make_float4(1.f, 1.f, 1.f, 1.f); gs[jv] = make_float4(0.f, 0.f, 0.f, 0.f);
        if (gscale && jv < nv) {
            ga[jv] = *reinterpret_cast<const float4*>(gscale + (size_t)b * C_in + 4 * (q + 4 * jv));
            gs[jv] = *reinterpret_cast<const float4*>(gshift + (size_t)b * C_in + 4 * (q + 4 * jv));
        }
    }
    __syncthreads();
    for (int r0 = 0; r0 < TW; r0 += 64) {
        const int r = r0 + (threadIdx.x >> 2);
        if (r < TW) {
            const int t = t0 - PAD + r;
            float acc[NP];
#pragma unroll
            for (int i = 0; i < NP; ++i) acc[i] = 0.f;
            if (t >= 0 && t < T) {
                const float* xr = x + ((size_t)b * T + t) * C_in;
#pragma unroll
                for (int jv = 0; jv < MAXV; ++jv) {
                    if (jv < nv) {
                        const int c4 = q + 4 * jv;
                        const float4 v4 = *reinterpret_cast<const float4*>(xr + 4 * c4);
                        float v[4] = {v4.x, v4.y, v4.z, v4.w};
                        if (gscale) {
                            const float a[4] = {ga[jv].x, ga[jv].y, ga[jv].z, ga[jv].w};
                            const float sh[4] = {gs[jv].x, gs[jv].y, gs[jv].z, gs[jv].w};
#pragma unroll
                            for (int e = 0; e < 4; ++e) v[e] = silu_f(fmaf(a[e], v[e], sh[e]));
                        }
#pragma unroll
                        for (int e = 0; e < 4; ++e) {
                            const float4* wr = reinterpret_cast<const float4*>(wl + (size_t)(4 * c4 + e) * NP);
#pragma unroll
                            for (int i4 = 0; i4 < NP / 4; ++i4) {
                                const float4 ww = wr[i4];
                                acc[4 * i4 + 0] = fmaf(ww.x, v[e], acc[4 * i4 + 0]);
                                acc[4 * i4 + 1] = fmaf(ww.y, v[e], acc[4 * i4 + 1]);
                                acc[4 * i4 + 2] = fmaf(ww.z, v[e], acc[4 * i4 + 2]);
                                acc[4 * i4 + 3] = fmaf(ww.w, v[e], acc[4 * i4 + 3]);
                            }
                        }
                    }
                }
            }
#pragma unroll
            for (int i = 0; i < NP; ++i) {
                acc[i] += __shfl_xor(acc[i], 1);
                acc[i] += __shfl_xor(acc[i], 2);
            }
            if (q == 0) {
                float4* pr = reinterpret_cast<float4*>(part + (size_t)r * NP);
#pragma unroll
                for (int i4 = 0; i4 < NP / 4; ++i4) pr[i4] = make_float4(acc[4 * i4], acc[4 * i4 + 1], acc[4 * i4 + 2], acc[4 * i4 + 3]);
            }
        }
    }
    __syncthreads();
    for (int o = threadIdx.x; o < 128 * C_out; o += 256) {
        const int co = o >> 7, tl = o & 127;
        const int t = t0 + tl;
        if (tl < NOUT && t < T) {
            float v = bias ? bias[co] : 0.f;
#pragma unroll
            for (int k = 0; k < KT; ++k) v += part[(size_t)(tl + k) * NP + k * MAXCO + co];
            const size_t oo = ((size_t)b * C_out + co) * T + t;
            if (c_out) v = v * c_out[b] + c_skip[b] * skip_src[oo];
            y[oo] = v;
        }
    }
}
}

namespace {
template <int KT, int NCO>
__global__ __launch_bounds__(256) void head_conv_row_kernel(const float* __restrict__ x, const float* __restrict__ gscale,
                                                            const float* __restrict__ gshift, const float* __restrict__ w,
                                                            const float* __restrict__ bias, const float* __restrict__ c_out,
                                                            const float* __restrict__ c_skip, const float* __restrict__ skip_src,
                                                            float* __restrict__ y, int T, int C_in, int ntiles, int co0, int C_tot) {
    constexpr int PAD = KT / 2, NOUT = 64 - (KT - 1), NP = KT * NCO;
    static_assert(NCO >= 1 && NCO <= 8, "a wave emits at most two output channels");
    extern __shared__ __attribute__((aligned(16))) float shm[];
    const int RS = C_in + 4;
    float* tile = shm;
    float* part = shm;
    const int lane = threadIdx.x & 63;
    const int wave = __builtin_amdgcn_readfirstlane((int)(threadIdx.x >> 6));
    const int b = blockIdx.x / ntiles, t0 = (blockIdx.x % ntiles) * NOUT;
    const int to = t0 + lane;
    const bool emit_t = lane < NOUT && to < T;
    size_t oo[2];
    float skipv[2] = {0.f, 0.f};
#pragma unroll
    for (int h = 0; h < 2; ++h) {
        const int co = wave + 4 * h;
        oo[h] = ((size_t)b * C_tot + co0 + (co < NCO ? co : 0)) * T + (to < T ? to : 0);
        if (c_out && emit_t && co < NCO) skipv[h] = skip_src[oo[h]];
    }
    {
        const int ncol = C_in >> 2, rpp = 256 / ncol;
        const int c4 = threadIdx.x % ncol, r0 = threadIdx.x / ncol;
        float4 a4 = make_float4(1.f, 1.f, 1.f, 1.f), s4 = make_float4(0.f, 0.f, 0.f, 0.f);
        if (gscale) {
            a4 = *reinterpret_cast<const float4*>(gscale + (size_t)b * C_in + 4 * c4);
            s4 = *reinterpret_cast<const float4*>(gshift + (size_t)b * C_in + 4 * c4);
        }
        const float* xb = x + (size_t)b * T * C_in + 4 * c4;
        for (int r = r0; r < 64; r += rpp) {
            const int t = t0 - PAD + r;
            float4 u = make_float4(0.f, 0.f, 0.f, 0.f);
            if (t >= 0 && t < T) {
                u = *reinterpret_cast<const float4*>(xb + (size_t)t * C_in);
                if (gscale) {
                    u.x = silu_f(fmaf(a4.x, u.x, s4.x)); u.y = silu_f(fmaf(a4.y, u.y, s4.y));
                    u.z = silu_f(fmaf(a4.z, u.z, s4.z)); u.w = silu_f(fmaf(a4.w, u.w, s4.w));
                }
            }
            *reinterpret_cast<float4*>(tile + r * RS + 4 * c4) = u;
        }
    }
    __syncthreads();
    const int cq = C_in >> 2;
    const float* ur = tile + lane * RS + wave * cq;
    float acc[KT][NCO];
#pragma unroll
    for (int k = 0; k < KT; ++k)
#pragma unroll
        for (int co = 0; co < NCO; ++co) acc[k][co] = 0.f;
    const float* wc[NCO];
#pragma unroll
    for (int co = 0; co < NCO; ++co) wc[co] = w + ((size_t)(co0 + co) * C_in + wave * cq) * KT;
#pragma unroll 1
    for (int c4 = 0; c4 < (cq >> 2); ++c4) {
        const float4 v4 = *reinterpret_cast<const float4*>(ur + 4 * c4);
        const float u[4] = {v4.x, v4.y, v4.z, v4.w};
#pragma unroll
        for (int co = 0; co < NCO; ++co) {
            const float* wr = wc[co] + 4 * c4 * KT;
#pragma unroll
            for (int e = 0; e < 4; ++e)
#pragma unroll
                for (int k = 0; k < KT; ++k) acc[k][co] = fmaf(wr[e * KT + k], u[e], acc[k][co]);
        }
    }
    __syncthreads();
#pragma unroll
    for (int k = 0; k < KT; ++k)
#pragma unroll
        for (int co = 0; co < NCO; ++co) {
            float* pr = part + ((wave * NP) + k * NCO + co) * 68;
            pr[lane] = acc[k][co];
            if (lane < 4) pr[64 + lane] = 0.f;
        }
    __syncthreads();
#pragma unroll
    for (int h = 0; h < (NCO > 4 ? 2 : 1); ++h) {
        const int co = wave + 4 * h;
        if (emit_t && co < NCO) {
            float v = bias ? bias[co0 + co] : 0.f;
#pragma unroll
            for (int k = 0; k < KT; ++k)
#pragma unroll
                for (int wv = 0; wv < 4; ++wv) v += part[((wv * NP) + k * NCO + co) * 68 + lane + k];
            if (c_out) v = v * c_out[b] + c_skip[b] * skipv[h];
            y[oo[h]] = v;
        }
    }
}
}

static size_t head_conv_lds(int C_in, int C_out, int ktaps) {
    if (C_in < 16 || C_in % 16 || C_in > 128 || C_out < 1 || C_out > 16 || (ktaps != 1 && ktaps != 3 && ktaps != 5)) return 0;
    const int maxco = C_out <= 4 ? 4 : 16;
    const size_t sh = ((size_t)C_in * ktaps * maxco + (size_t)128 * ktaps * maxco) * sizeof(float);
    return sh > 64 * 1024 ? 0 : sh;
}

extern "C" size_t tq_head_conv_lds_bytes(int C_in, int C_out, int ktaps) {
    const size_t sh = head_conv_lds(C_in, C_out, ktaps);
    return sh ? sh : ends_wide_head_fwd_lds(C_in, C_out, ktaps);
}

extern "C" size_t tq_stem_conv_lds_bytes(int C_in, int C_out, int ktaps) {
    if (ktaps != 1 && ktaps != 3 && ktaps != 5) return 0;
    if (!(C_in <= 0 || C_in > 16 || C_out < 4 || C_out % 4 || C_out > 1024 || 256 % (C_out / 4))) {
        const int nrow = 256 / (C_out / 4);
        const size_t sh = ((size_t)C_in * (STAT_SLOT + ktaps - 1) + (size_t)ktaps * C_in * C_out + (size_t)nrow * C_out * 2) * sizeof(float);
        if (sh <= 160 * 1024) return sh;
    }
    return ends_wide_stem_lds(C_in, C_out, ktaps);
}

extern "C" int tq_head_conv_fwd(const float* x, const float* gscale, const float* gshift, const float* w, const float* bias,
                                const float* c_out, const float* c_skip, const float* skip_src, float* y, int B, int T,
                                int C_in, int C_out, int ktaps, hipStream_t stream) {
    if (!x || !w || !y) return TQ_ERR_ARG;
    if ((gscale == nullptr) != (gshift == nullptr)) return TQ_ERR_ARG;
    if (c_out && (!c_skip || !skip_src)) return TQ_ERR_ARG;
    const size_t sh = head_conv_lds(C_in, C_out, ktaps);
    if (B <= 0 || T <= 0) return TQ_ERR_SHAPE;
    if (sh == 0) return ends_wide_head_fwd(x, gscale, gshift, w, bias, c_out, c_skip, skip_src, y, B, T, C_in, C_out, ktaps, stream);
    if ((C_out <= 4 || C_out == 6 || C_out == 8 || C_out == 16) && (C_in == 16 || C_in == 32 || C_in == 64 || C_in == 128)) {
        const int nt = (T + (64 - (ktaps - 1)) - 1) / (64 - (ktaps - 1));
        const int per = C_out <= 8 ? C_out : 8;
        const size_t st_ = (size_t)64 * (C_in + 4), sp_ = (size_t)4 * ktaps * per * 68;
        const size_t shr = (st_ > sp_ ? st_ : sp_) * sizeof(float);
#define TQ_HEADR(K, N, CO0) hipLaunchKernelGGL((head_conv_row_kernel<K, N>), dim3(B * nt), dim3(256), shr, stream, x, gscale, gshift, w, bias, \
                                               c_out, c_skip, skip_src, y, T, C_in, nt, CO0, C_out)
#define TQ_HEADRK(K) { if (per == 1) TQ_HEADR(K, 1, 0); else if (per == 2) TQ_HEADR(K, 2, 0); else if (per == 3) TQ_HEADR(K, 3, 0); \
                       else if (per == 4) TQ_HEADR(K, 4, 0); else if (per == 6) TQ_HEADR(K, 6, 0); \
                       else { for (int c0 = 0; c0 < C_out; c0 += 8) TQ_HEADR(K, 8, c0); } }
        if (ktaps == 5) TQ_HEADRK(5)
        else if (ktaps == 3) TQ_HEADRK(3)
        else TQ_HEADRK(1)
#undef TQ_HEADRK
#undef TQ_HEADR
        TQ_CHECK_LAUNCH();
        return 0;
    }
    const int nout = 128 - (ktaps - 1);
    const int ntiles = (T + nout - 1) / nout;
    const int maxco = C_out <= 4 ? 4 : 16;
#define TQ_HEAD(K)                                                                                          \
    {                                                                                                       \
        auto kern = (maxco == 4) ? head_conv_kernel<K, 4> : head_conv_kernel<K, 16>;                        \
        hipLaunchKernelGGL(kern, dim3(B * ntiles), dim3(256), sh, stream, x, gscale, gshift, w, bias, c_out, c_skip, skip_src, y, T, C_in, C_out, ntiles); \
    }
    if (ktaps == 5) TQ_HEAD(5)
    else if (ktaps == 3) TQ_HEAD(3)
    else if (ktaps == 1) TQ_HEAD(1)
    else return TQ_ERR_SHAPE;
#undef TQ_HEAD
    TQ_CHECK_LAUNCH();
    return 0;
}

namespace {
__device__ __forceinline__ void gemv_rows(const float* __restrict__ w, const float* __restrict__ bias,
                                          const float* in_sh, int n_in, int n_out, float* out_sh, bool accumulate) {
    const int tid = threadIdx.x;
    const int LPO = (n_in > 64 && (n_in & 15) == 0) ? 4 : 1;
    const int r = tid % LPO, o_local = tid / LPO;
    const int per_pass = 256 / LPO;
    const bool vec = (n_in & 3) == 0;
    for (int o0 = 0; o0 < n_out; o0 += per_pass) {
        const int o = o0 + o_local;
        float a = 0.f;
        if (o < n_out) {
            const float* wr = w + (size_t)o * n_in;
            if (vec) {
                const int n4 = n_in >> 2;
#pragma unroll 4
                for (int q = r; q < n4; q += LPO) {
                    const float4 wv = *reinterpret_cast<const float4*>(wr + 4 * q);
                    const float4 xv = *reinterpret_cast<const float4*>(in_sh + 4 * q);
                    a += wv.x * xv.x + wv.y * xv.y + wv.z * xv.z + wv.w * xv.w;
                }
            } else {
                for (int i = r; i < n_in; i += LPO) a = fmaf(wr[i], in_sh[i], a);
            }
        }
        for (int sft = 1; sft < LPO; sft <<= 1) a += __shfl_xor(a, sft);
        if (o < n_out && r == 0) {
            const float v = a + bias[o];
            out_sh[o] = accumulate ? out_sh[o] + v : v;
        }
    }
}

__global__ __launch_bounds__(256) void embed_kernel(const float* __restrict__ t, const float* __restrict__ cond,
                                                    const float* __restrict__ fw, const float* __restrict__ w0,
                                                    const float* __restrict__ b0, const float* __restrict__ w2,
                                                    const float* __restrict__ b2, const float* __restrict__ cw0,
                                                    const float* __restrict__ cb0, const float* __restrict__ cw2,
                                                    const float* __restrict__ cb2, float* __restrict__ emb,
                                                    float* __restrict__ silu_emb, float* __restrict__ hidden, int mc,
                                                    int ncond) {
    extern __shared__ __attribute__((aligned(16))) float shm[];
    const int E = 4 * mc;
    float* four = shm;
    float* h = four + mc;
    float* c = h + E;
    float* e = c + E;
    float* cs = e + E / 4;
    const int b = blockIdx.x, q = blockIdx.y;
    const float tv = t[b];
    const int half = mc >> 1;
    for (int i = threadIdx.x; i < half; i += 256) {
        const float arg = ((tv * fw[i]) * 2.0f) * 3.14159265358979323846f;
        four[i] = sinf(arg);
        four[half + i] = cosf(arg);
    }
    for (int i = threadIdx.x; i < ncond; i += 256) cs[i] = cond[(size_t)b * ncond + i];
    __syncthreads();
    gemv_rows(w0, b0, four, mc, E, h, false);
    if (ncond > 0) gemv_rows(cw0, cb0, cs, ncond, E, c, false);
    __syncthreads();
    for (int i = threadIdx.x; i < E; i += 256) {
        if (hidden && q == 0) {
            hidden[((size_t)b * 2 + 0) * E + i] = h[i];
            if (ncond > 0) hidden[((size_t)b * 2 + 1) * E + i] = c[i];
        }
        h[i] = silu_f(h[i]);
        if (ncond > 0) c[i] = silu_f(c[i]);
    }
    __syncthreads();
    const int o0 = q * (E / 4);
    gemv_rows(w2 + (size_t)o0 * E, b2 + o0, h, E, E / 4, e, false);
    if (ncond > 0) {
        __syncthreads();
        gemv_rows(cw2 + (size_t)o0 * E, cb2 + o0, c, E, E / 4, e, true);
    }
    __syncthreads();
    for (int i = threadIdx.x; i < E / 4; i += 256) {
        emb[(size_t)b * E + o0 + i] = e[i];
        silu_emb[(size_t)b * E + o0 + i] = silu_f(e[i]);
    }
// ... 741 lines not shown
```

tqdne_amd/engine.py:

```python

from __future__ import annotations

import ctypes as C
import os
from typing import List, Optional, Sequence, Tuple

import torch

from . import _lib
from .engine_bwd import BackwardPlan
from ._lib import (TQ_CONV_DROPOUT, TQ_CONV_EMB, TQ_CONV_GN, TQ_CONV_RES, TQ_CONV_SILU, TQ_CONV_STATS, STAT_SLOT,
                   TqConvDesc, _p, check)


def require_device(x: torch.Tensor):
    if not x.is_cuda:
        raise RuntimeError(
            "tqdne_amd runs its hot path on MI355X HIP kernels only; got a CPU tensor. "
            "(The CPU restatement lives in oracle/ and is test infrastructure, not a fallback.)"
        )
    if x.dtype != torch.float32:
        raise TypeError("tqdne_amd expects fp32 tensors at the boundary, like the reference (precision 32)")


def _noop_launch(*_args):
    return 0


def nslots(T: int) -> int:
    return (T + STAT_SLOT - 1) // STAT_SLOT


class Act:

    __slots__ = ("buf", "stats", "C", "T", "grad", "gw", "slot")

    def __init__(self, buf, stats, C, T, slot=STAT_SLOT):
        self.buf, self.stats, self.C, self.T = buf, stats, C, T
        self.slot = slot
        self.grad = None
        self.gw = False


FUSE_SKIP_CO = 32
SMALL_TILE_B = 4
SMALL_TILE_WGS = 64
GN_FOLD_DEFAULT = os.environ.get("TQDNE_GN_FOLD", "0") == "1"
CONCURRENT_LANE0 = 8


class ConvRec:

    __slots__ = ("site", "desc", "srcs", "gn", "out", "stride", "upsample", "silu", "dropout", "poly")

    def __init__(self, site, desc, srcs, gn, out, stride, upsample, silu, dropout):
        self.site, self.desc, self.srcs, self.gn, self.out = site, desc, srcs, gn, out
        self.stride, self.upsample, self.silu, self.dropout = stride, upsample, silu, dropout
        self.poly = None


_SIDE_STREAMS: dict = {}


def side_stream(dev, i: int = 1) -> "torch.cuda.Stream":
    key = (str(dev), i)
    s = _SIDE_STREAMS.get(key)
    if s is None:
        s = _SIDE_STREAMS[key] = torch.cuda.Stream(device=dev)
    return s


class lane_fanout:

    def __init__(self, dev, B: int, lanes: int):
        self.h = B // lanes
        self.main = torch.cuda.current_stream(dev)
        self.streams = [self.main] + [side_stream(dev, i) for i in range(1, lanes)]

    def rows(self, i: int) -> slice:
        return slice(i * self.h, (i + 1) * self.h)

    def cut(self, t, i: int):
        return None if t is None else t[self.rows(i)].contiguous()

    def __enter__(self):
        for st in self.streams[1:]:
            st.wait_stream(self.main)
        return self

    def __exit__(self, *exc):
        for st in self.streams[1:]:
            self.main.wait_stream(st)


def reserve_side_streams(dev, n: int = 3):
    if torch.device(dev).type != "cuda" or (str(dev), "reserved") in _SIDE_STREAMS or torch.cuda.is_current_stream_capturing():
        return
    _SIDE_STREAMS[(str(dev), "reserved")] = True
    import torch.distributed as dist
    if dist.is_available() and dist.is_initialized() and dist.get_backend() == "nccl":
        import warnings
        warnings.warn("tqdne_amd: the RCCL process group exists before this device's side streams made their first submission; if its "
                      "communicator is already created the backward's two streams may share a hardware queue (training step ~25 % "
                      "slower).  Call tqdne_amd.trainer.init_process_group(...) (or tqdne_amd.engine.reserve_side_streams(device)) "
                      "before torch.distributed.init_process_group.", RuntimeWarning, stacklevel=2)
    main = torch.cuda.current_stream(dev)
    z = torch.zeros(1, device=dev)
    for i in range(1, n + 1):
        s = side_stream(dev, i)
        s.wait_stream(main)
        with torch.cuda.stream(s):
            z.add_(0)
        main.wait_stream(s)


_PACK_TABLES: dict = {}


def pack_batch(lib, dev, jobs, stream, capturing=False):
    if not jobs:
        return
    key = (str(dev), tuple(jobs))
    ent = _PACK_TABLES.get(key)
    if ent is None and (capturing or len(jobs) < 2 or len(_PACK_TABLES) >= 4096):
        ent = False
    if ent is None:
        arr = (_lib.TqPackJob * len(jobs))()
        total = 0
        for jb, (src, dst, co, ci, k, mode) in zip(arr, jobs):
            jb.src, jb.dst, jb.C_out, jb.C_in, jb.K, jb.mode, jb.block_begin = src, dst, co, ci, k, mode, total
# ... 146 lines not shown
        flags[key] = torch.zeros(1, dtype=torch.int32, device=device)
    return flags[key]


def leave_fp16_range_scheme(model):
    model._conv_scheme = "bf16x3"
    for eng in getattr(model, "_engine_cache", {}).values():
        if eng.scheme == "auto":
            eng._set_scheme_bf16x3()


class Probe:

    def __init__(self, idx, name, flops):
        self.idx, self.name, self.flops, self.events = idx, name, flops, []

    def reset(self):
        self.events = []

    def result(self):
        if not self.events:
            return None, self.flops, self.name, 0
        torch.cuda.synchronize()
        ms = [a.elapsed_time(b) for a, b in self.events]
        return sum(ms) / len(ms), self.flops, self.name, len(ms)


_PLAN_UID = __import__("itertools").count(1)


class UNetEngine:
    def __init__(self, model, B: int, T: int, device: torch.device, solo: bool = True):
        self.lib = _lib.load()
        self.m = model
        self.B, self.T, self.dev = B, T, device
        self.solo = solo
        reserve_side_streams(device)
        self.store = get_store(model, device)
        self._seen_pack = {}
        self._clean_tag = None
        self.E = 4 * getattr(model, "model_channels", 0)
        self._keep = []
        self.ops: List[Tuple] = []
        self.ops_infer: List[Tuple] = []
        self.op_bytes: List[int] = []
        self.scheme = "auto"
        self.plan_epoch = 0
        self.uid = next(_PLAN_UID)
        self._wfmt_sites = []
        self.kv_v_format = _lib.attn_v_format()
        self._vfmt_ops = []
        self.ckpt = bool(getattr(model, "use_checkpoint", False))
        self._ckpt_pool = {}
        self._attn_train_ops = []
        self._block_kv = False
        self.range_flag = shared_range_flag(model, device)
        self._range_host = torch.zeros(1, dtype=torch.int32).pin_memory() if device.type == "cuda" else torch.zeros(1, dtype=torch.int32)
        self._range_evt = None
        self._range_held = False
        self._trace = None
        self.conv_sites: List[ConvSite] = []
        self.poly_sites: List[Tuple[ConvSite, ConvSite]] = []
        self.dropout_descs: List[TqConvDesc] = []
        self.acts: List[Act] = []
        self._probe = None
        self.tape = []
        self.last_rec = None
        self._bwd = None
        self.dgrad_sites = []
        self._wt_version = None
        self._last = None
        self._fwd_count = 0
        self._site_counter = 0
        self._pending_gn = None
        self._fold_default_ops = []
        self.gn_folded = 0
        self._last_poly_desc = None
        self._attn_ws = self._attn_ws_hd = None
        self.res_blocks, self.emb_offsets, self.emb_total = [], {}, 0
        self.emb_desc, self.emb_entry, self.emb_pack_mode, self.cond_four = None, None, 0, None
        self.wide_stem = self.wide_head = False
        self.x_btc = self.stem_out = self.stem_rec = None
        self.final = self.head_gn = self.head_btc = self.head_rec = self.out_nct = None
        self.out_mode = "head"
        self._build()
        assert self._pending_gn is None, "a deferred GroupNorm finalisation was never placed"
        if getattr(model, "_conv_scheme", "auto") == "bf16x3":
            self._set_scheme_bf16x3()

    def _empty(self, *shape, dtype=torch.float32):
        t = torch.empty(*shape, dtype=dtype, device=self.dev)
        self._keep.append(t)
        return t

    def _act(self, C_: int, T_: int, stats: bool = True, slot: int = STAT_SLOT) -> Act:
        a = Act(self._empty(self.B, T_, C_), self._empty(self.B, (T_ + slot - 1) // slot, C_, 2) if stats else None, C_, T_, slot)
        self.acts.append(a)
        return a

    def _ckpt_act(self, tag: str, C_: int, T_: int, stats: bool = True, slot: int = STAT_SLOT) -> Act:
        key = (tag, C_, T_, stats, slot)
        first = self._ckpt_pool.get(key)
        if first is None:
            first = self._ckpt_pool[key] = self._act(C_, T_, stats, slot)
            return first
        a = Act(first.buf, first.stats, C_, T_, slot)
        self.acts.append(a)
        return a

    def _site(self, name: str, conv: torch.nn.Module, pad_cin=None, pad_cout=None) -> ConvSite:
        s = ConvSite(name, conv.weight, conv.bias, self.dev, self.lib, store=self.store, pad_cin=pad_cin, pad_cout=pad_cout)
        self.conv_sites.append(s)
        return s

    def _site_pair(self, name: str, conv, tail_name: str, tail_conv):
        lib = self.lib
        co, ci, k = conv.weight.shape
        tco, tci, tk = tail_conv.weight.shape
        assert tk == 1 and tco == co
        main_bytes = lib.tq_conv_weight_pack_bytes(co, ci, k, 0)
        tail_bytes = lib.tq_conv_weight_pack_bytes(tco, tci, 1, 0)
        s = ConvSite(name, conv.weight, conv.bias, self.dev, lib, tail_bytes=tail_bytes, store=self.store)
        t = ConvSite(tail_name, tail_conv.weight, tail_conv.bias, self.dev, lib, packed=s.packed[main_bytes:])
        s.tail = t
        self.conv_sites += [s, t]
        return s, t

    def _emit(self, op, infer_op=None, nbytes=0):
        self.ops.append(op)
        self.ops_infer.append(op if infer_op is None else infer_op)
        self.op_bytes.append(nbytes)

    def _launch_bound(self, T_out: int) -> bool:
        return self.B <= SMALL_TILE_B or (self.solo and self.B * ((T_out + 127) // 128) <= SMALL_TILE_WGS)

    def _gn(self, srcs: Sequence[Act], norm: torch.nn.GroupNorm, defer: bool = False):
        C_ = sum(s.C for s in srcs)
        gscale, gshift = self._empty(self.B, C_), self._empty(self.B, C_)
        mean_rstd = self._empty(self.B, 32, 2)
        s0 = srcs[0]
        s1 = srcs[1] if len(srcs) > 1 else None
        fin = ((self.lib.tq_gn_finalize, (
            _p(s0.stats), s0.C, _p(s1.stats) if s1 else None, s1.C if s1 else 0, self.B, s0.T,
            _p(norm.weight), _p(norm.bias), _p(gscale), _p(gshift), _p(mean_rstd), s0.slot, s1.slot if s1 else 0), "gn_finalize", 0),
            4 * self.B * (2 * nslots(s0.T) * C_ + 2 * C_))
        if defer:
            self._pending_gn = dict(key=gscale.data_ptr(), fin=fin, srcs=(s0, s1), norm=norm, mean_rstd=mean_rstd)
            return gscale, gshift, mean_rstd
        self._emit(fin[0], nbytes=fin[1])
        return gscale, gshift, mean_rstd

    def _conv(self, srcs: Sequence[Act], site: ConvSite, *, gn=None, silu=False, emb_ptr=None, res: Optional[Act] = None,
              stats=True, stride=1, upsample=False, dropout_site: Optional[int] = None, launch: bool = True,
              skip: Optional[Tuple[Sequence[Act], ConvSite]] = None, qkv_planes=None, ckpt_tag: Optional[str] = None) -> Optional[Act]:
        s0 = srcs[0]
        s1 = srcs[1] if len(srcs) > 1 else None
        if s1 is not None and s1.T != s0.T:
            raise RuntimeError(f"Sizes of tensors must match except in dimension 1: lengths {s0.T} and {s1.T} at {site.name} "
                               "(the signal length must be divisible by the UNet's total down-sampling factor)")
        T_in = s0.T
        if stride == 2:
            T_out = (T_in + 2 - site.K) // 2 + 1
            pad = site.K // 2
        else:
            T_out = 2 * T_in if upsample else T_in
            pad = site.K // 2
        srcs_c = [s0.C, (s1.C if s1 else 0)] + ([a.C for a in skip[0]] if skip is not None else [])
        k5_act = site.K == 5 and gn is not None and silu and stride == 1 and not upsample and qkv_planes is None
        _check_width_limits(site.name, site.C_in, site.C_out)
        wfmt = _lib.forward_wfmt(site.C_out, srcs_c, stride, upsample, k5_act=k5_act, gn=gn is not None) if launch else 0
        small = (launch and self._launch_bound(T_out) and k5_act
                 and wfmt in (_lib.TQ_WFMT_BF16X3, _lib.TQ_WFMT_F16_MX6))
        if small and wfmt == _lib.TQ_WFMT_F16_MX6 and site.C_out % 128:
            wfmt = _lib.TQ_WFMT_BF16X3
        if launch and ckpt_tag is not None and self.ckpt:
            out = self._ckpt_act(ckpt_tag, site.C_out, T_out, stats, slot=32 if small else STAT_SLOT)
        else:
            out = self._act(site.C_out, T_out, stats, slot=32 if small else STAT_SLOT) if launch else None
        d = TqConvDesc()
        d.t_tile = 32 if small else 0
        pend = self._pending_gn
        if pend is not None and gn is not None and pend["key"] == gn[0].data_ptr():
            self._pending_gn = None
            fold_max = self.lib.tq_conv1d_gn_fold_max_cin(wfmt, 32 if small else 0, site.C_out)
            if small and wfmt != _lib.TQ_WFMT_BF16X3:
                fold_max = min(fold_max, self.lib.tq_conv1d_gn_fold_max_cin(_lib.TQ_WFMT_BF16X3, 32, site.C_out))
            fold_fits = site.C_in <= fold_max
            fold_default = (GN_FOLD_DEFAULT and not small and k5_act and wfmt == _lib.TQ_WFMT_F16_MX6 and self.scheme == "auto"
                            and getattr(self.m, "_conv_scheme", "auto") == "auto" and fold_fits)
            if fold_default and launch and not self.ckpt:
                fn, fargs, fname, ffl = pend["fin"][0]
                self._fold_default_ops.append((len(self.ops), fn, d))
                self._emit((_noop_launch, fargs, fname + " (folded into its consumer)", ffl), nbytes=0)
            if launch and ((small and fold_fits) or fold_default) and not self.ckpt:
                f = _lib.TqGnFold()
                ps0, ps1 = pend["srcs"]
                f.stats0, f.stats1 = _p(ps0.stats), (_p(ps1.stats) if ps1 is not None else None)
                f.slot0, f.slot1 = ps0.slot, (ps1.slot if ps1 is not None else 0)
                f.gamma, f.beta, f.mean_rstd = _p(pend["norm"].weight), _p(pend["norm"].bias), _p(pend["mean_rstd"])
                self._keep.append(f)
                d.gn_fold = C.pointer(f)
                self.gn_folded += 1
            else:
                self._emit(pend["fin"][0], nbytes=pend["fin"][1])
        d.B, d.T_in, d.T_out = self.B, T_in, T_out
        d.C_in0, d.C_in1, d.C_out = s0.C, (s1.C if s1 else 0), site.C_out
        assert d.C_in0 + d.C_in1 == site.C_in, (site.name, d.C_in0, d.C_in1, site.C_in)
        d.ktaps, d.stride, d.pad, d.upsample = site.K, stride, pad, int(upsample)
        flags = 0
        if gn is not None:
            flags |= TQ_CONV_GN
        if silu:
            flags |= TQ_CONV_SILU
        if emb_ptr is not None:
            flags |= TQ_CONV_EMB
        if res is not None:
            flags |= TQ_CONV_RES
            assert res.C == site.C_out and res.T == T_out
        if stats:
            flags |= TQ_CONV_STATS
        if site.K == 1 and self._launch_bound(T_out):
            flags |= _lib.TQ_CONV_CH_TILES
        d.flags = flags
        d.emb_stride = self.emb_total
        d.wfmt = wfmt
        if launch:
            site.pack_mode = _lib.PACK_MODE[d.wfmt]
            if skip is not None:
                skip[1].pack_mode = site.pack_mode
            self._wfmt_sites.append((d, [site] + ([skip[1]] if skip is not None else []), d.wfmt))
            if stats:
                d.range_flag = self.range_flag.data_ptr()
        d.dropout_site = dropout_site or 0
        d.dropout_p = 0.0
        d.dropout_seed = 0
        if dropout_site is not None:
            self.dropout_descs.append(d)
        self._keep.append(d)
        flops = 2 * site.C_in * site.C_out * site.K * T_out * self.B
        nbytes = 4 * self.B * (T_in * site.C_in + T_out * site.C_out + (T_out * site.C_out if res is not None else 0))
        if skip is not None:
            ksrcs, ksite = skip
            k0, k1 = ksrcs[0], (ksrcs[1] if len(ksrcs) > 1 else None)
            assert res is None and k0.T == T_out and ksite.C_out == site.C_out
            d.C_skip0, d.C_skip1 = k0.C, (k1.C if k1 else 0)
            self._emit((self.lib.tq_conv1d_fwd_skip, (
                C.byref(d), _p(s0.buf), _p(s1.buf) if s1 else None, _p(gn[0]) if gn else None, _p(gn[1]) if gn else None,
                _p(site.packed), _p(site.bias), emb_ptr, _p(k0.buf), _p(k1.buf) if k1 else None, _p(ksite.bias),
                _p(out.buf), _p(out.stats)),
                "conv:" + site.name + "+skip", flops + 2 * ksite.C_in * site.C_out * T_out * self.B),
                nbytes=nbytes + 4 * self.B * T_out * ksite.C_in)
        elif launch:
            op = (self.lib.tq_conv1d_fwd, (
                C.byref(d), _p(s0.buf), _p(s1.buf) if s1 else None, _p(gn[0]) if gn else None, _p(gn[1]) if gn else None,
                _p(site.packed), _p(site.bias_pad if site.bias_pad is not None else site.bias), emb_ptr, _p(res.buf) if res else None,
                _p(out.buf), _p(out.stats)), "conv:" + site.name, flops)
            infer_op = None
            if (upsample and site.K == 5 and (T_in % STAT_SLOT == 0 or T_in % STAT_SLOT > STAT_SLOT // 2) and site.C_out % 32 == 0 and gn is None and res is None
                    and emb_ptr is None and os.environ.get("TQDNE_POLYPHASE_UPSAMPLE", "1") != "0"):
                infer_op = self._polyphase_op(site, d, s0, s1, out, flops)
                if s1 is None:
                    op = infer_op
            if qkv_planes is not None:
                ws, H_, D_ = qkv_planes
                d.range_flag = self.range_flag.data_ptr()
                infer_op = (self.lib.tq_conv1d_fwd_qkv, (
                    C.byref(d), _p(s0.buf), _p(gn[0]) if gn else None, _p(gn[1]) if gn else None, _p(site.packed), _p(site.bias),
                    _p(out.buf), _p(ws), H_, D_, self.kv_v_format), "conv:" + site.name + "+split", flops)
                self._vfmt_ops.append(len(self.ops_infer))
            self._emit(op, infer_op, nbytes=nbytes)
        self.last_rec = ConvRec(site, d, list(srcs), gn, out, stride, upsample, silu, dropout_site is not None)
        if launch and upsample and s1 is None and self.poly_sites and self.poly_sites[-1][1] is site:
            self.last_rec.poly = (self.poly_sites[-1][0], self._last_poly_desc)
        return out

    def _resample_plain(self, x: Act, name: str, up: bool) -> Act:
        if x.C % 4 or x.C > 1024 or x.T < 2:
            raise NotImplementedError(f"{name}: parameter-free resampling of a ({x.T}, {x.C}) tensor; the HIP kernels take 4 | C <= 1024 and "
                                      "at least two positions")
        out = self._act(x.C, 2 * x.T if up else x.T // 2, True)
        fn, what = (self.lib.tq_nearest_up2_fwd, "nearest_up2:") if up else (self.lib.tq_avg_pool2_fwd, "avg_pool2:")
        self._emit((fn, (_p(x.buf), _p(out.buf), _p(out.stats), self.B, x.T, x.C), what + name, 0),
                   nbytes=4 * self.B * x.C * (x.T + out.T))
        self.tape.append(("up_plain" if up else "down_plain", dict(x=x, out=out)))
        return out

    def _polyphase_op(self, site: ConvSite, d: TqConvDesc, s0: Act, s1: Optional[Act], out: Act, flops: int):
        Cr = site.C_out
        w2 = self.store.entry("w:" + site.name + ":polyphase", (2 * Cr, site.C_in, 3), torch.float32)["buf"]
        ps = ConvSite(site.name + ":polyphase", w2, site.bias, self.dev, self.lib, store=self.store)
        self.poly_sites.append((ps, site))
        d2 = TqConvDesc()
        d2.B, d2.T_in, d2.T_out = d.B, d.T_in, d.T_in
        d2.C_in0, d2.C_in1, d2.C_out = d.C_in0, d.C_in1, 2 * Cr
        d2.ktaps, d2.stride, d2.pad, d2.upsample = 3, 1, 1, 0
        d2.flags = (d.flags & TQ_CONV_STATS) | _lib.TQ_CONV_POLY2
        d2.emb_stride = 0
        d2.wfmt = _lib.forward_wfmt(2 * Cr, [d.C_in0, d.C_in1], gn=False)
        ps.pack_mode = _lib.PACK_MODE[d2.wfmt]
        self._wfmt_sites.append((d2, [ps], d2.wfmt))
        if d2.flags & TQ_CONV_STATS:
            d2.range_flag = self.range_flag.data_ptr()
        self._keep.append(d2)
        self._last_poly_desc = d2
        return (self.lib.tq_conv1d_fwd, (
            C.byref(d2), _p(s0.buf), _p(s1.buf) if s1 else None, None, None, _p(ps.packed), _p(site.bias), None, None,
            _p(out.buf), _p(out.stats)), "conv:" + site.name + "+polyphase", flops)

    def _build(self):
        m, B, T = self.m, self.B, self.T
        lib = self.lib
        self.res_blocks = []
        for blk in list(m.input_blocks) + [m.middle_block] + list(m.output_blocks):
            for layer in blk:
                if getattr(layer, "kind", None) == "res":
                    self.res_blocks.append(layer)
        self.emb_offsets = {}
        off = 0
        for rb in self.res_blocks:
            self.emb_offsets[id(rb)] = off
            off += rb.out_channels
        self.emb_total = off
        self.emb = self._empty(B, self.E)
        self.silu_emb = self._empty(B, self.E)
        self.emb_hidden = self._empty(B, 2, self.E)
        self.emb_w = self.store.entry("emb_w", (self.emb_total, self.E), torch.float32)["buf"]
        self.emb_b = self.store.entry("emb_b", (self.emb_total,), torch.float32)["buf"]
        if self.emb_total > 0 and self.E % 32 == 0 and self.emb_total % 32 == 0:
            d = TqConvDesc()
            d.B, d.T_in, d.T_out, d.C_in0, d.C_in1, d.C_out = 1, B, B, self.E, 0, self.emb_total
            d.ktaps, d.stride, d.pad, d.upsample, d.flags = 1, 1, 0, 0, 0
            d.wfmt = _lib.forward_wfmt(self.emb_total, [self.E], gn=False)
            self.emb_pack_mode = _lib.PACK_MODE[d.wfmt]
            self.emb_entry = self.store.entry("emb_packed", lib.tq_conv_weight_pack_bytes(self.emb_total, self.E, 1, self.emb_pack_mode))
            self.emb_packed = self.emb_entry["buf"]
            self._keep.append(d)
            self.emb_desc = d
        self.emb_all = self._empty(B, self.emb_total)
        self.cond_four = self._empty(B, m.model_channels) if getattr(m, "cond_embed", None) is not None else None

        stem = m.input_blocks[0][0]
        self._stem(stem, m.in_channels, T, "input_blocks.0.0")
        hs = [self.stem_out]
        h = self.stem_out
        for i, blk in enumerate(m.input_blocks):
            if i == 0:
                continue
            h = self._layers(blk, h, f"input_blocks.{i}")
            hs.append(h)
        h = self._layers(m.middle_block, h, "middle_block")
        for i, blk in enumerate(m.output_blocks):
            skip = hs.pop()
            h = self._layers(blk, (h, skip), f"output_blocks.{i}")
        self.final = h
        self.wide_head = m.out[2].out_channels > NARROW_SIGNAL_CHANNELS
        if not self.wide_head:
            _check_head_limits(h.C, m.out[2].out_channels, m.out[2].kernel_size[0])
        self.head_gn = self._gn([h], m.out[0])
        if self.wide_head:
            self.out_mode = "wide"
            self._wide_head(h, m.out[2], "out.2", self.head_gn)
        self.out_nct = self._empty(B, m.out_channels, T)

    def _layers(self, layers, h, name: str):
        for li, layer in enumerate(layers):
            kind = getattr(layer, "kind", None)
            pfx = f"{name}.{li}"
            if kind == "res":
                h = self._res_block(h, layer, pfx)
            elif kind == "attn":
                h = self._attention(h[0] if isinstance(h, tuple) else h, layer, pfx)
            elif kind == "down" and not layer.use_conv:
                h = self._resample_plain(h, pfx, up=False)
            elif kind == "up" and not layer.use_conv:
                h = self._resample_plain(h, pfx, up=True)
            elif kind == "down":
                x_in = h
                h = self._conv([h], self._site(pfx + ".op", layer.op), stride=2)
                self.tape.append(("down", dict(x=x_in, out=h, rec=self.last_rec)))
            elif kind == "up":
                x_in = h
                h = self._conv([h], self._site(pfx + ".conv", layer.conv), upsample=True)
                self.tape.append(("up", dict(x=x_in, out=h, rec=self.last_rec)))
            else:
                raise RuntimeError(f"unexpected layer {type(layer)} in {name}")
        return h

    def _stem(self, stem, cin: int, T: int, name: str):
        self.wide_stem = cin > NARROW_SIGNAL_CHANNELS
        if not self.wide_stem:
            _check_stem_limits(cin, stem.out_channels, stem.kernel_size[0], name)
            self.stem_out = self._act(stem.out_channels, T, True)
            return
        _check_boundary_limits("input conv", name, cin, stem.kernel_size[0])
        self.x_btc = self._act((cin + 31) // 32 * 32, T, stats=False)
        self.stem_out = self._conv([self.x_btc], self._site(name, stem, pad_cin=self.x_btc.C), stats=True)
        self.stem_rec = self.last_rec

    def _wide_head(self, h: Act, conv, name: str, gn):
        _check_boundary_limits("output conv", name, conv.out_channels, conv.kernel_size[0])
        site = self._site(name, conv, pad_cout=(conv.out_channels + 31) // 32 * 32)
        self.head_btc = self._conv([h], site, gn=gn, silu=gn is not None, stats=False)
        self.head_rec = self.last_rec

    def _run_stem(self, x, in_scale, stem, cin, stream, trace, what, name, cond_x=None):
        B, T, co, K = self.B, self.T, stem.out_channels, stem.kernel_size[0]
        e0 = _recorded_event() if trace is not None else None
        if self.wide_stem:
            c1 = 0 if cond_x is None else cond_x.shape[1]
            check(self.lib.tq_nct_to_btc(_p(x), _p(in_scale), _p(cond_x), _p(self.x_btc.buf), B, cin - c1, c1, T, self.x_btc.C,
                                         stream), what + " (nct_to_btc)")
            entry = ("nct_to_btc:" + name, 0, 4 * B * T * (cin + self.x_btc.C))
        else:
            check(self.lib.tq_stem_conv_fwd(_p(x), _p(in_scale), _p(stem.weight), _p(stem.bias), _p(self.stem_out.buf),
                                            _p(self.stem_out.stats), B, cin, T, co, K, stream), what)
            entry = (name, 2 * B * T * cin * co * K, 4 * B * T * (cin + co))
        if trace is not None:
            trace.append(entry + (e0, _recorded_event()))

    def _run_head(self, head, epilogue, stream, trace, what, name):
        B, T, fin, co, K = self.B, self.final.T, self.final, head.out_channels, head.kernel_size[0]
        c_out, c_skip, skip_src = epilogue or (None, None, None)
        io = co * (1 if epilogue is None else 2)
        e0 = _recorded_event() if trace is not None else None
        if self.out_mode == "head":
            gn = self.head_gn or (None, None)
            check(self.lib.tq_head_conv_fwd(_p(fin.buf), _p(gn[0]), _p(gn[1]), _p(head.weight), _p(head.bias), _p(c_out), _p(c_skip),
                                            _p(skip_src), _p(self.out_nct), B, T, fin.C, co, K, stream), what)
            entry = (name, 2 * B * T * fin.C * co * K, 4 * B * T * (fin.C + io))
        elif self.out_mode == "wide":
            check(self.lib.tq_btc_to_nct(_p(self.head_btc.buf), _p(c_out), _p(c_skip), _p(skip_src), _p(self.out_nct), B, T,
                                         self.head_btc.C, 0, co, stream), "head epilogue (btc_to_nct)")
            entry = ("btc_to_nct:" + name, 0, 4 * B * T * (self.head_btc.C + io))
        else:
            self.out_nct.copy_(self.head_btc.buf.permute(0, 2, 1))
            entry = ("output layout flip", 0, 4 * B * T * (fin.C + io))
        if trace is not None:
            trace.append(entry + (e0, _recorded_event()))

    def _arm_dropout(self, p: float, seed: int, descs=None, flag: int = TQ_CONV_DROPOUT):
        for d in self.dropout_descs if descs is None else descs:
            if p > 0.0:
                d.flags |= flag
                d.dropout_p, d.dropout_seed = p, seed
            else:
                d.flags &= ~flag

    def _run_ops(self, ops, stream, trace):
        probe = self._probe
        if trace is None and (probe is None or torch.cuda.is_current_stream_capturing()):
            for fn, args, what, _ in ops:
                rc = fn(*args, stream)
                if rc:
                    check(rc, what)
            return
        for i, (fn, args, what, fl) in enumerate(ops):
            timed = trace is not None or i == probe.idx
            a = _recorded_event() if timed else None
            rc = fn(*args, stream)
            if trace is not None:
                trace.append((what, fl, self.op_bytes[i], a, _recorded_event()))
            elif timed:
                probe.events.append((a, _recorded_event()))
            if rc:
                check(rc, what)

    def _res_block(self, x, rb, name: str) -> Act:
        srcs = list(x) if isinstance(x, tuple) else [x]
        emb_ptr = self.emb_all.data_ptr() + 4 * self.emb_offsets[id(rb)] if hasattr(rb, "emb_layers") else None
        g1 = self._gn(srcs, rb.in_layers[0], defer=not self.ckpt)
        i_conv1 = len(self.ops)
        h1 = self._conv(srcs, self._site(name + ".in_layers.2", rb.in_layers[2]), gn=g1, silu=True, emb_ptr=emb_ptr, ckpt_tag="h1")
        rec1 = self.last_rec
        i_gn2 = len(self.ops)
        g2 = self._gn([h1], rb.out_layers[0], defer=not self.ckpt)
        recompute = list(range(i_conv1, len(self.ops))) if self.ckpt else None
        rec_sk = None
        conv2 = rb.out_layers[3]
        self._site_counter += 1
        if isinstance(rb.skip_connection, torch.nn.Identity):
            assert len(srcs) == 1
            out = self._conv([h1], self._site(name + ".out_layers.3", conv2), gn=g2, silu=True, res=srcs[0],
                             dropout_site=self._site_counter)
        elif conv2.weight.shape[2] == 5 and conv2.weight.shape[0] % FUSE_SKIP_CO == 0 and all(a.C % 32 == 0 for a in srcs):
            site2, site_sk = self._site_pair(name + ".out_layers.3", conv2, name + ".skip_connection", rb.skip_connection)
            self._conv(srcs, site_sk, stats=False, launch=False)
            rec_sk = self.last_rec
            out = self._conv([h1], site2, gn=g2, silu=True, dropout_site=self._site_counter, skip=(srcs, site_sk))
        else:
            res = self._conv(srcs, self._site(name + ".skip_connection", rb.skip_connection), stats=False)
            rec_sk = self.last_rec
            out = self._conv([h1], self._site(name + ".out_layers.3", conv2), gn=g2, silu=True, res=res,
                             dropout_site=self._site_counter)
        self.tape.append(("res", dict(rb=rb, srcs=srcs, g1=g1, g2=g2, h1=h1, out=out, rec1=rec1, rec2=self.last_rec,
                                      rec_sk=rec_sk, recompute=recompute)))
        return out

    def _attention(self, x: Act, ab, name: str) -> Act:
        g = self._gn([x], ab.norm)
        D = ab.channels // ab.num_heads
        hd = D not in (32, 64, 128)
        if hd and not self.lib.tq_attention_head_tile(D):
            raise NotImplementedError(f"attention head dim {D}: kernels exist for multiples of 8 from 8 to 256 "
                                      "(larger heads need another kernel structure: their K / V tiles do not fit the LDS)")
        ws_bytes = self.lib.tq_attention_hd_workspace_bytes if hd else self.lib.tq_attention_workspace_bytes
        ws = self._attn_workspace(ws_bytes(self.B, x.T, ab.num_heads, D), "_attn_ws_hd" if hd else "_attn_ws")
        split = (ws, ab.num_heads, D) if D in (32, 64) else None
        i_qkv = len(self.ops)
        qkv = self._conv([x], self._site(name + ".qkv", ab.qkv), gn=g, silu=False, stats=False, qkv_planes=split, ckpt_tag="qkv")
        rec_qkv = self.last_rec
        att = self._ckpt_act("att", ab.channels, x.T, False) if self.ckpt else self._act(ab.channels, x.T, False)
        if self.ckpt:
            lse = self._ckpt_pool.get(("lse", ab.num_heads, x.T))
            if lse is None:
                lse = self._ckpt_pool[("lse", ab.num_heads, x.T)] = self._empty(self.B, ab.num_heads, x.T)
        else:
            lse = self._empty(self.B, ab.num_heads, x.T)
        flops = 4 * ab.channels * x.T * x.T * self.B
        fwd = self.lib.tq_attention_fwd_hd if hd else self.lib.tq_attention_fwd
        ws_fwd = ws if (split is not None or self._launch_bound(x.T)) else None
        op = (fwd, (_p(qkv.buf), _p(att.buf), _p(lse), _p(ws_fwd), self.B, x.T, ab.num_heads, D), "attention", flops)
        if split is not None and not self.ckpt:
            self._attn_train_ops.append((len(self.ops), len(self.tape), ws.numel()))
        infer_op = None
        if split is not None:
            infer_op = (self.lib.tq_attention_fwd_presplit, (_p(qkv.buf), _p(ws), _p(att.buf), self.B, x.T, ab.num_heads, D,
                                                             self.kv_v_format), "attention", flops)
            self._vfmt_ops.append(len(self.ops_infer))
        self._emit(op, infer_op, nbytes=4 * self.B * x.T * 4 * ab.channels)
        recompute = list(range(i_qkv, len(self.ops))) if self.ckpt else None
        out = self._conv([att], self._site(name + ".proj_out", ab.proj_out), res=x)
        entry = dict(ab=ab, x=x, g=g, qkv=qkv, att=att, lse=lse, out=out, rec_qkv=rec_qkv, rec_proj=self.last_rec, D=D,
                     recompute=recompute)
        if self.ckpt and split is not None:
            entry["kv_ws"], entry["kv_always"] = ws, True
        self.tape.append(("attn", entry))
        return out

    def _attn_workspace(self, nbytes: int, slot: str = "_attn_ws"):
        ws = getattr(self, slot)
        if ws is None or ws.numel() != nbytes:
            ws = torch.zeros(nbytes, dtype=torch.uint8, device=self.dev)
            self._keep.append(ws)
            setattr(self, slot, ws)
        return ws

    def install_probe(self, name_prefix: str = "conv:"):
        idx = max((i for i, op in enumerate(self.ops) if op[2].startswith(name_prefix)), key=lambda i: self.ops[i][3])
        self._probe = Probe(idx, self.ops[idx][2], self.ops[idx][3])
        return self._probe

    def _set_scheme_bf16x3(self):
        for d, sites, _pref in self._wfmt_sites:
            d.wfmt = _lib.TQ_WFMT_BF16X3
            for st in sites:
                st.pack_mode = 0
        for i, fn, d in self._fold_default_ops:
            for ops in (self.ops, self.ops_infer):
                _f, a_, w_, fl_ = ops[i]
                ops[i] = (fn, a_, "gn_finalize", fl_)
            d.gn_fold = None
        self._fold_default_ops = []
        if self.emb_desc is not None:
            self.emb_desc.wfmt = _lib.TQ_WFMT_BF16X3
            self.emb_pack_mode = 0
        self.set_kv_v_format(_lib.TQ_KV_V_BF16)
        self.scheme = "bf16x3"
        self.plan_epoch += 1

    def enable_block_kv(self):
        if self._block_kv:
            return
        for i, ti, nbytes in self._attn_train_ops:
            ws = torch.zeros(nbytes, dtype=torch.uint8, device=self.dev)
            self._keep.append(ws)
            fn, args, *rest = self.ops[i]
            self.ops[i] = (fn, args[:3] + (ws.data_ptr(),) + args[4:], *rest)
            self.tape[ti][1]["kv_ws"] = ws
        self._block_kv = True

    def set_kv_v_format(self, fmt: int):
        if fmt != self.kv_v_format:
# ... 280 lines not shown
```

tqdne_amd/ops.py:

```python

from __future__ import annotations

import ctypes as C
from typing import Optional, Tuple

import torch

from . import _lib
from ._lib import (TQ_CONV_DROPOUT, TQ_CONV_EMB, TQ_CONV_GN, TQ_CONV_RES, TQ_CONV_SILU, TQ_CONV_STATS, STAT_SLOT,
                   TqConvDesc, _p, check)


def _stream(dev):
    return torch.cuda.current_stream(dev).cuda_stream


def nslots(T):
    return (T + STAT_SLOT - 1) // STAT_SLOT


def pack_conv_weight(w: torch.Tensor, mode: int = 0, geometry=None) -> torch.Tensor:
    lib = _lib.load()
    co, ci, k = w.shape
    gco, gci = geometry or (co, ci)
    assert gco >= co and gci >= ci and (gco - co) < 32 and (gci - ci) < 32
    out = torch.empty(lib.tq_conv_weight_pack_bytes(gco, gci, k, mode), dtype=torch.uint8, device=w.device)
    check(lib.tq_pack_conv_weight(_p(w.contiguous()), co, ci, k, mode, _p(out), _stream(w.device)), "pack")
    return out


def conv1d(x0, weight, bias=None, *, x1=None, gscale=None, gshift=None, silu=False, emb=None, residual=None,
           stride=1, upsample=False, stats=True, dropout_p=0.0, dropout_seed=0, dropout_site=0, skip=None, wfmt=None, t_tile=0,
           gn_fold=None, wide_table=False, out=None, pad_cout=0):
    lib = _lib.load()
    B, T_in, C0 = x0.shape
    C1 = 0 if x1 is None else x1.shape[2]
    w_co, C_in, K = weight.shape
    C_out = pad_cout or w_co
    assert C_in == C0 + C1 or (x1 is None and skip is None and 0 < C0 - C_in < 32)
    assert not pad_cout or bias is None or bias.numel() == C_out
    T_out = (T_in + 2 * (K // 2) - K) // 2 + 1 if stride == 2 else (2 * T_in if upsample else T_in)
    if out is not None:
        y, st = out
        stats = st is not None
    else:
        y = torch.empty(B, T_out, C_out, device=x0.device)
        st = torch.empty(B, (T_out + 31) // 32 if t_tile == 32 else nslots(T_out), C_out, 2, device=x0.device) if stats else None
    d = TqConvDesc()
    d.B, d.T_in, d.T_out, d.C_in0, d.C_in1, d.C_out = B, T_in, T_out, C0, C1, C_out
    d.ktaps, d.stride, d.pad, d.upsample = K, stride, K // 2, int(upsample)
    d.t_tile = t_tile
    f = 0
    if gscale is not None:
        f |= TQ_CONV_GN
    if silu:
        f |= TQ_CONV_SILU
    if emb is not None:
        f |= TQ_CONV_EMB
    if residual is not None:
        f |= TQ_CONV_RES
    if stats:
        f |= TQ_CONV_STATS
    if dropout_p > 0:
        f |= TQ_CONV_DROPOUT
    if wide_table:
        f |= _lib.TQ_CONV_WIDE_TABLE
    d.flags = f
    d.emb_stride = 0 if emb is None else emb.stride(0)
    d.dropout_site, d.dropout_p, d.dropout_seed = dropout_site, dropout_p, dropout_seed
    if wfmt is None:
        srcs = [C0, C1] + ([skip[0].shape[2], 0 if skip[1] is None else skip[1].shape[2]] if skip is not None else [])
        wfmt = _lib.forward_wfmt(C_out, srcs, stride, upsample,
                                 k5_act=K == 5 and gscale is not None and silu and stride == 1 and not upsample and t_tile == 0,
                                 gn=gscale is not None)
    d.wfmt = wfmt
    if gn_fold is not None:
        f = _lib.TqGnFold()
        f.stats0, f.stats1, f.slot0, f.slot1 = _p(gn_fold[0]), _p(gn_fold[1]), gn_fold[2], gn_fold[3]
        f.gamma, f.beta, f.mean_rstd = _p(gn_fold[4]), _p(gn_fold[5]), _p(gn_fold[6])
        d.gn_fold = C.pointer(f)
    pmode = _lib.PACK_MODE[wfmt]
    wp = pack_conv_weight(weight, pmode, geometry=(C_out, C0 + C1))
    if skip is not None:
        sx0, sx1, wsk, bsk = skip
        assert residual is None
        d.C_skip0, d.C_skip1 = sx0.shape[2], (0 if sx1 is None else sx1.shape[2])
        wp = torch.cat([wp, pack_conv_weight(wsk, pmode)])
        check(lib.tq_conv1d_fwd_skip(C.byref(d), _p(x0), _p(x1), _p(gscale), _p(gshift), _p(wp), _p(bias), _p(emb), _p(sx0),
                                     _p(sx1), _p(bsk), _p(y), _p(st), _stream(x0.device)), "conv1d_skip")
        return y, st
    check(lib.tq_conv1d_fwd(C.byref(d), _p(x0), _p(x1), _p(gscale), _p(gshift), _p(wp), _p(bias), _p(emb), _p(residual),
                            _p(y), _p(st), _stream(x0.device)), "conv1d")
    return y, st


def gn_finalize(stats0, C0, T, gamma, beta, stats1=None, C1=0, slot0=0, slot1=0):
    lib = _lib.load()
    B = stats0.shape[0]
    Cn = C0 + C1
    gs, gh = torch.empty(B, Cn, device=gamma.device), torch.empty(B, Cn, device=gamma.device)
    mr = torch.empty(B, 32, 2, device=gamma.device)
    check(lib.tq_gn_finalize(_p(stats0), C0, _p(stats1), C1, B, T, _p(gamma), _p(beta), _p(gs), _p(gh), _p(mr), slot0, slot1,
                             _stream(gamma.device)), "gn_finalize")
    return gs, gh, mr


def stem_conv(x_nct, weight, bias, in_scale=None, stats=True, out=None):
    lib = _lib.load()
    B, Cin, T = x_nct.shape
    Cout, _, K = weight.shape
    if out is not None:
        y, st = out
    else:
        y = torch.empty(B, T, Cout, device=x_nct.device)
        st = torch.empty(B, nslots(T), Cout, 2, device=x_nct.device) if stats else None
    check(lib.tq_stem_conv_fwd(_p(x_nct.contiguous()), _p(in_scale), _p(weight.contiguous()), _p(bias), _p(y), _p(st), B, Cin,
                               T, Cout, K, _stream(x_nct.device)), "stem")
    return y, st


def head_conv(x, weight, bias, gscale=None, gshift=None, c_out=None, c_skip=None, skip_src=None, out=None):
    lib = _lib.load()
    B, T, Cin = x.shape
    Cout, _, K = weight.shape
    y = torch.empty(B, Cout, T, device=x.device) if out is None else out
    check(lib.tq_head_conv_fwd(_p(x), _p(gscale), _p(gshift), _p(weight.contiguous()), _p(bias), _p(c_out), _p(c_skip),
                               _p(skip_src), _p(y), B, T, Cin, Cout, K, _stream(x.device)), "head")
    return y


def nct_to_btc(x_nct, scale=None, cond_nct=None, Cp=None, out=None):
    lib = _lib.load()
    B, C0, T = x_nct.shape
    C1 = 0 if cond_nct is None else cond_nct.shape[1]
    if Cp is None:
        Cp = (C0 + C1 + 31) // 32 * 32 if out is None else out.shape[2]
    y = torch.empty(B, T, Cp, device=x_nct.device) if out is None else out
    check(lib.tq_nct_to_btc(_p(x_nct.contiguous()), _p(scale), _p(None if cond_nct is None else cond_nct.contiguous()), _p(y), B, C0, C1,
                            T, Cp, _stream(x_nct.device)), "nct_to_btc")
    return y


def btc_to_nct(v_btc, C, c_off=0, a=None, s=None, skip_src=None, out=None):
    lib = _lib.load()
    B, T, Cp = v_btc.shape
    y = torch.empty(B, C, T, device=v_btc.device) if out is None else out
    check(lib.tq_btc_to_nct(_p(v_btc), _p(a), _p(s), _p(skip_src), _p(y), B, T, Cp, c_off, C, _stream(v_btc.device)), "btc_to_nct")
    return y

# ... 262 lines not shown
```

Measured before the change: 354.3.

## Fold GroupNorm finalisation into bf16x3 and pointwise consumer convs by default

Extends the in-kernel GroupNorm-statistics fold, which computes scale/shift inside the consuming conv, from the f16mx6 k=5 path to bf16x3 tiles (TBW 8) and to pointwise k=1 convs. It places the coefficient table inside a staging buffer and delays the table store in the pointwise path until after the fold. The fold is turned on by default, attention GroupNorm is deferred so it can fold, and an opt-in fold for the head conv is added. This removes separate gn_finalize launches and their round trips. In exchange every consumer workgroup redoes the per-sample statistics reduction, and the table shares LDS with staging.

```diff
diff --git a/include/tqdne_hip.h b/include/tqdne_hip.h
--- a/include/tqdne_hip.h
+++ b/include/tqdne_hip.h
@@ -26,6 +26,7 @@
 #define TQ_CONV_POLY2 64
 #define TQ_CONV_CH_TILES 128
 #define TQ_CONV_WIDE_TABLE 256
+#define TQ_CONV_FOLD_BF16X3 512
 
 #define TQ_WFMT_BF16X3 0
 #define TQ_WFMT_F16_MX8 1
@@ -91,6 +92,7 @@
 size_t tq_conv1d_wide_lds_bytes(int ktaps, int t_tile, int C_out);
 int tq_conv1d_gn_table_entries(int wide);
 int tq_conv1d_gn_fold_max_cin(int wfmt, int t_tile, int C_out);
+int tq_conv1d_gn_fold_max_cin_flags(int wfmt, int t_tile, int C_out, int flags);
 int tq_colsum_max_channels(void);
 typedef struct TqPackJob {
     const void* src;
@@ -134,6 +136,10 @@
 int tq_head_conv_fwd(const float* x, const float* gscale, const float* gshift, const float* w, const float* bias,
                      const float* c_out, const float* c_skip, const float* skip_src, float* y_nct, int B, int T, int C_in,
                      int C_out, int ktaps, hipStream_t stream);
+int tq_head_conv_folds(int C_in, int C_out, int ktaps);
+int tq_head_conv_fwd_fold(const float* x, const TqGnFold* fold, float* gscale, float* gshift, const float* w, const float* bias,
+                          const float* c_out, const float* c_skip, const float* skip_src, float* y_nct, int B, int T, int C_in,
+                          int C_out, int ktaps, hipStream_t stream);
 
 int tq_gn_finalize(const float* stats0, int C0, const float* stats1, int C1, int B, int T, const float* gamma,
                    const float* beta, float* gscale, float* gshift, float* mean_rstd, int slot0, int slot1, hipStream_t stream);
diff --git a/tqdne_amd/_lib.py b/tqdne_amd/_lib.py
--- a/tqdne_amd/_lib.py
+++ b/tqdne_amd/_lib.py
@@ -19,6 +19,7 @@
 TQ_CONV_POLY2 = 64
 TQ_CONV_CH_TILES = 128
 TQ_CONV_WIDE_TABLE = 256
+TQ_CONV_FOLD_BF16X3 = 512
 TQ_WFMT_BF16X3, TQ_WFMT_F16_MX8, TQ_WFMT_F16_MX6 = 0, 1, 2
 TQ_KV_V_BF16, TQ_KV_V_F16 = 0, 1
 PACK_MODE = {TQ_WFMT_BF16X3: 0, TQ_WFMT_F16_MX8: 2, TQ_WFMT_F16_MX6: 3}
@@ -128,11 +129,14 @@
     "tq_conv1d_gn_table_entries": (I, [I]),
     "tq_conv1d_wide_lds_bytes": (SZ, [I, I, I]),
     "tq_conv1d_gn_fold_max_cin": (I, [I, I, I]),
+    "tq_conv1d_gn_fold_max_cin_flags": (I, [I, I, I, I]),
     "tq_colsum_max_channels": (I, []),
     "tq_conv1d_fwd": (I, [C.POINTER(TqConvDesc)] + [VP] * 11),
     "tq_conv1d_fwd_skip": (I, [C.POINTER(TqConvDesc)] + [VP] * 13),
     "tq_stem_conv_fwd": (I, [VP] * 6 + [I] * 5 + [VP]),
     "tq_head_conv_fwd": (I, [VP] * 9 + [I] * 5 + [VP]),
+    "tq_head_conv_folds": (I, [I, I, I]),
+    "tq_head_conv_fwd_fold": (I, [VP, C.POINTER(TqGnFold)] + [VP] * 8 + [I] * 5 + [VP]),
     "tq_head_conv_lds_bytes": (SZ, [I, I, I]),
     "tq_stem_conv_lds_bytes": (SZ, [I, I, I]),
     "tq_head_conv_bwd_lds_bytes": (SZ, [I, I, I]),
diff --git a/tqdne_amd/csrc/conv1d_fwd_wide.hip b/tqdne_amd/csrc/conv1d_fwd_wide.hip
--- a/tqdne_amd/csrc/conv1d_fwd_wide.hip
+++ b/tqdne_amd/csrc/conv1d_fwd_wide.hip
@@ -61,7 +61,14 @@
 
 extern "C" int tq_conv1d_max_cout(void) { return 3 * CONV_GTAB_NARROW; }
 
-extern "C" int tq_conv1d_gn_fold_max_cin(int wfmt, int t_tile, int C_out) {
+template <int WM, int WN, int SCH>
+static constexpr int fold_max_default() {
+    constexpr int k1 = ConvLds<1, 1, 0, WM, WN, 0, 1, SCH, false, 8, 2, 1024>::FOLD_MAX_CIN;
+    constexpr int k5 = ConvLds<5, 1, 0, WM, WN, 0, 2, SCH, false, 8, 2, 1024>::FOLD_MAX_CIN;
+    return k1 < k5 ? k1 : k5;
+}
+
+extern "C" int tq_conv1d_gn_fold_max_cin_flags(int wfmt, int t_tile, int C_out, int flags) {
     if (C_out <= 0 || C_out % 32) return 0;
     int lim = 0;
     if (t_tile == 32) {
@@ -71,8 +78,15 @@
         else if (C_out % 64 == 0) lim = ConvLds<5, 1, 0, 2, 1, 0, 2, 0, false, 2, 2, 1024>::FOLD_MAX_CIN;
         else lim = ConvLds<5, 1, 0, 1, 1, 0, 2, 0, false, 2, 2, 1024>::FOLD_MAX_CIN;
     } else if (t_tile == 0 && wfmt == TQ_WFMT_F16_MX6) {
-        if (C_out % 256 == 0) lim = ConvLds<5, 1, 0, 8, 1, 0, 2, 2, false, 8, 2, 1024>::FOLD_MAX_CIN;
-        else if (C_out % 128 == 0) lim = ConvLds<5, 1, 0, 4, 1, 0, 2, 2, false, 8, 2, 1024>::FOLD_MAX_CIN;
+        if (C_out % 256 == 0) lim = fold_max_default<8, 1, 2>();
+        else if (C_out % 128 == 0) lim = fold_max_default<4, 1, 2>();
+    } else if (t_tile == 0 && wfmt == TQ_WFMT_BF16X3 && (flags & TQ_CONV_FOLD_BF16X3)) {
+        if (C_out % 256 == 0) lim = fold_max_default<8, 1, 0>();
+        else if (C_out % 128 == 0) lim = fold_max_default<4, 1, 0>();
+        else if (C_out % 64 == 0) lim = fold_max_default<2, 2, 0>();
+        else lim = fold_max_default<1, 2, 0>();
     }
     return lim / 32 * 32;
 }
+
+extern "C" int tq_conv1d_gn_fold_max_cin(int wfmt, int t_tile, int C_out) { return tq_conv1d_gn_fold_max_cin_flags(wfmt, t_tile, C_out, 0); }
diff --git a/tqdne_amd/csrc/conv1d_kernel.hpp b/tqdne_amd/csrc/conv1d_kernel.hpp
--- a/tqdne_amd/csrc/conv1d_kernel.hpp
+++ b/tqdne_amd/csrc/conv1d_kernel.hpp
@@ -243,8 +243,10 @@
     float nlog2e = -1.4426950408889634f, n4096 = -4096.f;
     asm volatile("" : "+s"(nlog2e), "+s"(n4096));
 
-    float* gtab = reinterpret_cast<float*>(lds + (PW ? 4 * C::BUF : C::LDS_BYTES));
-    constexpr bool FOLD_LATE0 = SCH == 0 && TBW == 2 && ACT >= 1 && !PW && EPI == 0;
+    constexpr bool FOLD_LATE0 = SCH == 0 && (TBW == 2 || TBW == 8) && ACT >= 1 && !PW && (EPI == 0 || EPI == 2) && STRIDE == 1 && UPS == 0;
+    constexpr bool FOLD0_TAB_INSIDE = FOLD_LATE0 && TBW == 8;
+    static_assert(!FOLD0_TAB_INSIDE || C::BUF >= CONV_FOLD0_TAB_BYTES, "the table of the bf16x3 default tiles lies inside staging buffer 1");
+    float* gtab = reinterpret_cast<float*>(lds + (PW ? 4 * C::BUF : (FOLD0_TAB_INSIDE ? C::LDS_BYTES - CONV_FOLD0_TAB_BYTES : C::LDS_BYTES)));
     const bool fold0_pending = FOLD_LATE0 && p.cf_st0 != nullptr;
     auto chunk_base2 = [&](int stage, int& cs) -> const float* __attribute__((always_inline)) {
         const bool sk = FUSE && stage >= nchunks;
@@ -591,7 +593,7 @@
 
     static_assert(!(SCH == 2 && ACT >= 1) || C::NTHR >= 256, "one table entry per thread");
     constexpr int GT_N = GTW / 1024;
-    constexpr bool FOLD_LATE = SCH == 2 && ACT >= 1 && !PW && EPI == 0 && (TBW == 8 || TBW == 2);
+    constexpr bool FOLD_LATE = SCH == 2 && ACT >= 1 && (EPI == 0 || EPI == 2) && (TBW == 8 || TBW == 2);
     const bool fold_late = FOLD_LATE && p.cf_st0 != nullptr;
     float4 gt_a = make_float4(0.f, 0.f, 0.f, 0.f), gt_s = gt_a;
     int gt_i = 0;
@@ -633,7 +635,9 @@
             __syncthreads();
         }
     };
-    if constexpr (PW) gtab_store();
+    if constexpr (PW) {
+        if (!fold_late) gtab_store();
+    }
     const int npass = PW ? n_ctiles : 1;
     if constexpr (PW) {
         static_assert(!PW || SCH == 2 || C::NIT == C::PRE, "PW stages a chunk in PRE iterations");
@@ -646,8 +650,14 @@
                 const float* base2 = chunk_base2(c < nchunks ? c : nchunks - 1, cs2);
                 load16(base2, cs2, tid >> 2, rr2[c]);
             }
-            load_w(0, wa);
-            load_w(1, wb);
+            if (fold_late) {
+                gtab_store();
+                load_w(0, wa);
+                load_w(1, wb);
+            } else {
+                load_w(0, wa);
+                load_w(1, wb);
+            }
 #pragma unroll
             for (int c = 0; c < 4; ++c) write16(c < nchunks ? c : nchunks - 1, c, tid >> 2, rr2[c]);
             __syncthreads();
@@ -1095,7 +1105,8 @@
     static constexpr int GTAB_MAX = ((SCH == 2 && ACT >= 1) || (SCH == 0 && TBW == 2 && ACT >= 1 && !PW && EPI == 0)) ? 2 * 4 * GTW : 0;
     static constexpr int STAGE = PW ? 4 * C::BUF : C::LDS_BYTES;
     static constexpr int BYTES = STAGE + GTAB_MAX;
-    static constexpr int FOLD_MAX_CIN = GTW != 1024 ? 0 : ((STAGE / 8 - 64) / 2 < 1024 ? (STAGE / 8 - 64) / 2 : 1024);
+    static constexpr int FOLD_SCRATCH = STAGE - ((SCH == 0 && TBW == 8) ? CONV_FOLD0_TAB_BYTES : 0);
+    static constexpr int FOLD_MAX_CIN = GTW != 1024 ? 0 : ((FOLD_SCRATCH / 8 - 64) / 2 < 1024 ? (FOLD_SCRATCH / 8 - 64) / 2 : 1024);
 };
 constexpr int TQ_LDS_WORKGROUP_MAX = 163840;
 
@@ -1108,11 +1119,12 @@
     constexpr int LDS_BYTES = L::BYTES;
     static_assert(LDS_BYTES <= TQ_LDS_WORKGROUP_MAX, "tile + coefficient table exceed the LDS a workgroup may declare");
     if (a.cf_st0 && GTW != 1024) return TQ_ERR_SHAPE;
-    if (GTAB_MAX && a.cf_st0 && a.C0 + a.C1 > 1024) return TQ_ERR_SHAPE;
+    if (a.cf_st0 && a.C0 + a.C1 > 1024) return TQ_ERR_SHAPE;
     if (SCH == 2 && ACT >= 1 && a.C0 + a.C1 > GTW) return TQ_ERR_SHAPE;
     if (a.cf_st0) {
-        constexpr bool built = (TBW == 2 && ACT >= 1 && !PW && EPI == 0) || (SCH == 2 && ACT >= 1 && !PW && EPI == 0 && TBW == 8);
-        if (!built || (size_t)(2 * (a.C0 + a.C1) + 64) * sizeof(double) > (size_t)(LDS_BYTES - GTAB_MAX)) return TQ_ERR_SHAPE;
+        constexpr bool built = (EPI == 0 || EPI == 2) && ACT >= 1 && STRIDE == 1 && UPS == 0 &&
+                               ((SCH == 0 && !PW && (TBW == 2 || TBW == 8)) || (SCH == 2 && (TBW == 2 || TBW == 8)));
+        if (!built || (size_t)(2 * (a.C0 + a.C1) + 64) * sizeof(double) > (size_t)L::FOLD_SCRATCH) return TQ_ERR_SHAPE;
     }
     static std::atomic<uint64_t> attr_done{0};
     int dev_ord = 0;
diff --git a/tqdne_amd/csrc/conv1d_mfma.hip b/tqdne_amd/csrc/conv1d_mfma.hip
--- a/tqdne_amd/csrc/conv1d_mfma.hip
+++ b/tqdne_amd/csrc/conv1d_mfma.hip
@@ -106,7 +106,8 @@
     a.cf_st0 = a.cf_st1 = a.cf_gamma = a.cf_beta = nullptr; a.cf_mean_rstd = nullptr; a.cf_ns0 = a.cf_ns1 = 0;
     if (d->gn_fold) {
         const TqGnFold* f = d->gn_fold;
-        if (!(d->flags & TQ_CONV_GN) || kv_planes || (a.t_tile != 32 && d->wfmt != TQ_WFMT_F16_MX6)) return TQ_ERR_SHAPE;
+        if (!(d->flags & TQ_CONV_GN) || (a.t_tile != 32 && d->wfmt != TQ_WFMT_F16_MX6 && d->wfmt != TQ_WFMT_BF16X3)) return TQ_ERR_SHAPE;
+        if (a.t_tile != 32 && d->wfmt == TQ_WFMT_BF16X3 && !(d->flags & TQ_CONV_FOLD_BF16X3)) return TQ_ERR_SHAPE;
         if (!f->stats0 || !f->gamma || !f->beta || (d->C_in1 > 0 && !f->stats1)) return TQ_ERR_ARG;
         const int s0 = f->slot0 ? f->slot0 : STAT_SLOT, s1 = f->slot1 ? f->slot1 : STAT_SLOT;
         if ((s0 != STAT_SLOT && s0 != 32) || (s1 != STAT_SLOT && s1 != 32)) return TQ_ERR_ARG;
diff --git a/tqdne_amd/csrc/conv_args.hpp b/tqdne_amd/csrc/conv_args.hpp
--- a/tqdne_amd/csrc/conv_args.hpp
+++ b/tqdne_amd/csrc/conv_args.hpp
@@ -72,6 +72,7 @@
 int conv_launch_resample(const ConvArgs& a, int ktaps, int stride, hipStream_t stream);
 int conv_launch_dgrad(const ConvArgs& a, int ktaps, hipStream_t stream);
 constexpr int CONV_GTAB_NARROW = 1024, CONV_GTAB_WIDE = 2048;
+constexpr int CONV_FOLD0_TAB_BYTES = 2 * 4 * CONV_GTAB_NARROW;
 inline bool conv_wide_table(const ConvArgs& a) { return a.C0 + a.C1 > CONV_GTAB_NARROW || (a.flags & TQ_CONV_WIDE_TABLE); }
 int conv_launch_fwd_wide(const ConvArgs& a, int ktaps, int act, bool fuse, hipStream_t stream);
 int conv_launch_fwd_wide_k5(const ConvArgs& a, int act, bool fuse, hipStream_t stream);
diff --git a/tqdne_amd/csrc/small_ops.hip b/tqdne_amd/csrc/small_ops.hip
--- a/tqdne_amd/csrc/small_ops.hip
+++ b/tqdne_amd/csrc/small_ops.hip
@@ -159,12 +159,31 @@
 }
 
 namespace {
-template <int KT, int MAXCO>
+struct HeadFold {
+    const float* st;
+    const float* gamma;
+    const float* beta;
+    float* gscale;
+    float* gshift;
+    float* mean_rstd;
+    int nslots, lds_off;
+};
+__device__ __forceinline__ const float* head_fold(const HeadFold& hf, float* shm, int b, int T, int C_in) {
+    double* scratch = reinterpret_cast<double*>(shm + hf.lds_off);
+    float* tab = reinterpret_cast<float*>(scratch + 2 * C_in + 2 * GN_GROUPS);
+    gn_fold_sample<false, false>(scratch, b, hf.st, C_in, nullptr, 0, T, hf.nslots, 0, hf.gamma, hf.beta, hf.gscale, hf.gshift, hf.mean_rstd,
+                                 tab, tab + C_in);
+    __syncthreads();
+    return tab;
+}
+static size_t head_fold_lds(int C_in) { return (size_t)(2 * C_in + 2 * GN_GROUPS) * sizeof(double) + (size_t)2 * C_in * sizeof(float); }
+
+template <int KT, int MAXCO, bool FOLD = false>
 __global__ __launch_bounds__(256) void head_conv_kernel(const float* __restrict__ x, const float* __restrict__ gscale,
                                                         const float* __restrict__ gshift, const float* __restrict__ w,
                                                         const float* __restrict__ bias, const float* __restrict__ c_out,
                                                         const float* __restrict__ c_skip, const float* __restrict__ skip_src,
-                                                        float* __restrict__ y, int T, int C_in, int C_out, int ntiles) {
+                                                        float* __restrict__ y, int T, int C_in, int C_out, int ntiles, const HeadFold hf) {
     extern __shared__ __attribute__((aligned(16))) float shm[];
     constexpr int PAD = KT / 2;
     constexpr int TW = 128;
@@ -184,10 +203,17 @@
     const int q = threadIdx.x & 3;
     const int nv = C_in >> 4;
     float4 ga[MAXV], gs[MAXV];
+    const float* ftab = nullptr;
+    if constexpr (FOLD) ftab = head_fold(hf, shm, b, T, C_in);
 #pragma unroll
     for (int jv = 0; jv < MAXV; ++jv) {
         ga[jv] = make_float4(1.f, 1.f, 1.f, 1.f); gs[jv] = make_float4(0.f, 0.f, 0.f, 0.f);
-        if (gscale && jv < nv) {
+        if constexpr (FOLD) {
+            if (jv < nv) {
+                ga[jv] = *reinterpret_cast<const float4*>(ftab + 4 * (q + 4 * jv));
+                gs[jv] = *reinterpret_cast<const float4*>(ftab + C_in + 4 * (q + 4 * jv));
+            }
+        } else if (gscale && jv < nv) {
             ga[jv] = *reinterpret_cast<const float4*>(gscale + (size_t)b * C_in + 4 * (q + 4 * jv));
             gs[jv] = *reinterpret_cast<const float4*>(gshift + (size_t)b * C_in + 4 * (q + 4 * jv));
         }
@@ -258,12 +284,13 @@
 }
 
 namespace {
-template <int KT, int NCO>
+template <int KT, int NCO, bool FOLD = false>
 __global__ __launch_bounds__(256) void head_conv_row_kernel(const float* __restrict__ x, const float* __restrict__ gscale,
                                                             const float* __restrict__ gshift, const float* __restrict__ w,
                                                             const float* __restrict__ bias, const float* __restrict__ c_out,
                                                             const float* __restrict__ c_skip, const float* __restrict__ skip_src,
-                                                            float* __restrict__ y, int T, int C_in, int ntiles, int co0, int C_tot) {
+                                                            float* __restrict__ y, int T, int C_in, int ntiles, int co0, int C_tot,
+                                                            const HeadFold hf) {
     constexpr int PAD = KT / 2, NOUT = 64 - (KT - 1), NP = KT * NCO;
     static_assert(NCO >= 1 && NCO <= 8, "a wave emits at most two output channels");
     extern __shared__ __attribute__((aligned(16))) float shm[];
@@ -287,16 +314,24 @@
         const int ncol = C_in >> 2, rpp = 256 / ncol;
         const int c4 = threadIdx.x % ncol, r0 = threadIdx.x / ncol;
         float4 a4 = make_float4(1.f, 1.f, 1.f, 1.f), s4 = make_float4(0.f, 0.f, 0.f, 0.f);
-        if (gscale) {
+        const float* xb = x + (size_t)b * T * C_in + 4 * c4;
+        float4 first = make_float4(0.f, 0.f, 0.f, 0.f);
+        if constexpr (FOLD) {
+            const int tf = t0 - PAD + r0;
+            first = *reinterpret_cast<const float4*>(xb + (size_t)(tf < 0 ? 0 : (tf < T ? tf : T - 1)) * C_in);
+            const float* ftab = head_fold(hf, shm, b, T, C_in);
+            a4 = *reinterpret_cast<const float4*>(ftab + 4 * c4);
+            s4 = *reinterpret_cast<const float4*>(ftab + C_in + 4 * c4);
+        } else if (gscale) {
             a4 = *reinterpret_cast<const float4*>(gscale + (size_t)b * C_in + 4 * c4);
             s4 = *reinterpret_cast<const float4*>(gshift + (size_t)b * C_in + 4 * c4);
         }
-        const float* xb = x + (size_t)b * T * C_in + 4 * c4;
         for (int r = r0; r < 64; r += rpp) {
             const int t = t0 - PAD + r;
             float4 u = make_float4(0.f, 0.f, 0.f, 0.f);
             if (t >= 0 && t < T) {
-                u = *reinterpret_cast<const float4*>(xb + (size_t)t * C_in);
+                if (FOLD && r == r0) u = first;
+                else u = *reinterpret_cast<const float4*>(xb + (size_t)t * C_in);
                 if (gscale) {
                     u.x = silu_f(fmaf(a4.x, u.x, s4.x)); u.y = silu_f(fmaf(a4.y, u.y, s4.y));
                     u.z = silu_f(fmaf(a4.z, u.z, s4.z)); u.w = silu_f(fmaf(a4.w, u.w, s4.w));
@@ -377,22 +412,26 @@
     return ends_wide_stem_lds(C_in, C_out, ktaps);
 }
 
-extern "C" int tq_head_conv_fwd(const float* x, const float* gscale, const float* gshift, const float* w, const float* bias,
-                                const float* c_out, const float* c_skip, const float* skip_src, float* y, int B, int T,
-                                int C_in, int C_out, int ktaps, hipStream_t stream) {
-    if (!x || !w || !y) return TQ_ERR_ARG;
-    if ((gscale == nullptr) != (gshift == nullptr)) return TQ_ERR_ARG;
-    if (c_out && (!c_skip || !skip_src)) return TQ_ERR_ARG;
+template <bool FOLD>
+static int head_conv_launch(const float* x, const float* gscale, const float* gshift, const float* w, const float* bias,
+                            const float* c_out, const float* c_skip, const float* skip_src, float* y, int B, int T, int C_in,
+                            int C_out, int ktaps, HeadFold hf, hipStream_t stream) {
     const size_t sh = head_conv_lds(C_in, C_out, ktaps);
     if (B <= 0 || T <= 0) return TQ_ERR_SHAPE;
-    if (sh == 0) return ends_wide_head_fwd(x, gscale, gshift, w, bias, c_out, c_skip, skip_src, y, B, T, C_in, C_out, ktaps, stream);
+    if (sh == 0) {
+        if (FOLD) return TQ_ERR_SHAPE;
+        return ends_wide_head_fwd(x, gscale, gshift, w, bias, c_out, c_skip, skip_src, y, B, T, C_in, C_out, ktaps, stream);
+    }
+    const size_t fold_bytes = FOLD ? head_fold_lds(C_in) : 0;
     if ((C_out <= 4 || C_out == 6 || C_out == 8 || C_out == 16) && (C_in == 16 || C_in == 32 || C_in == 64 || C_in == 128)) {
         const int nt = (T + (64 - (ktaps - 1)) - 1) / (64 - (ktaps - 1));
         const int per = C_out <= 8 ? C_out : 8;
         const size_t st_ = (size_t)64 * (C_in + 4), sp_ = (size_t)4 * ktaps * per * 68;
-        const size_t shr = (st_ > sp_ ? st_ : sp_) * sizeof(float);
-#define TQ_HEADR(K, N, CO0) hipLaunchKernelGGL((head_conv_row_kernel<K, N>), dim3(B * nt), dim3(256), shr, stream, x, gscale, gshift, w, bias, \
-                                               c_out, c_skip, skip_src, y, T, C_in, nt, CO0, C_out)
+        const size_t shr0 = (st_ > sp_ ? st_ : sp_) * sizeof(float);
+        hf.lds_off = (int)((shr0 + 15) / 16 * 4);
+        const size_t shr = FOLD ? (size_t)hf.lds_off * sizeof(float) + fold_bytes : shr0;
+#define TQ_HEADR(K, N, CO0) hipLaunchKernelGGL((head_conv_row_kernel<K, N, FOLD>), dim3(B * nt), dim3(256), shr, stream, x, gscale, gshift, w, bias, \
+                                               c_out, c_skip, skip_src, y, T, C_in, nt, CO0, C_out, hf)
 #define TQ_HEADRK(K) { if (per == 1) TQ_HEADR(K, 1, 0); else if (per == 2) TQ_HEADR(K, 2, 0); else if (per == 3) TQ_HEADR(K, 3, 0); \
                        else if (per == 4) TQ_HEADR(K, 4, 0); else if (per == 6) TQ_HEADR(K, 6, 0); \
                        else { for (int c0 = 0; c0 < C_out; c0 += 8) TQ_HEADR(K, 8, c0); } }
@@ -407,10 +446,13 @@
     const int nout = 128 - (ktaps - 1);
     const int ntiles = (T + nout - 1) / nout;
     const int maxco = C_out <= 4 ? 4 : 16;
+    hf.lds_off = (int)((sh + 15) / 16 * 4);
+    const size_t shg = FOLD ? (size_t)hf.lds_off * sizeof(float) + fold_bytes : sh;
+    if (shg > 64 * 1024) return TQ_ERR_SHAPE;
 #define TQ_HEAD(K)                                                                                          \
     {                                                                                                       \
-        auto kern = (maxco == 4) ? head_conv_kernel<K, 4> : head_conv_kernel<K, 16>;                        \
-        hipLaunchKernelGGL(kern, dim3(B * ntiles), dim3(256), sh, stream, x, gscale, gshift, w, bias, c_out, c_skip, skip_src, y, T, C_in, C_out, ntiles); \
+        auto kern = (maxco == 4) ? head_conv_kernel<K, 4, FOLD> : head_conv_kernel<K, 16, FOLD>;            \
+        hipLaunchKernelGGL(kern, dim3(B * ntiles), dim3(256), shg, stream, x, gscale, gshift, w, bias, c_out, c_skip, skip_src, y, T, C_in, C_out, ntiles, hf); \
     }
     if (ktaps == 5) TQ_HEAD(5)
     else if (ktaps == 3) TQ_HEAD(3)
@@ -419,6 +461,38 @@
 #undef TQ_HEAD
     TQ_CHECK_LAUNCH();
     return 0;
+}
+
+extern "C" int tq_head_conv_fwd(const float* x, const float* gscale, const float* gshift, const float* w, const float* bias,
+                                const float* c_out, const float* c_skip, const float* skip_src, float* y, int B, int T,
+                                int C_in, int C_out, int ktaps, hipStream_t stream) {
+    if (!x || !w || !y) return TQ_ERR_ARG;
+    if ((gscale == nullptr) != (gshift == nullptr)) return TQ_ERR_ARG;
+    if (c_out && (!c_skip || !skip_src)) return TQ_ERR_ARG;
+    return head_conv_launch<false>(x, gscale, gshift, w, bias, c_out, c_skip, skip_src, y, B, T, C_in, C_out, ktaps, HeadFold{}, stream);
+}
+
+extern "C" int tq_head_conv_folds(int C_in, int C_out, int ktaps) {
+    const size_t sh = head_conv_lds(C_in, C_out, ktaps);
+    if (sh == 0 || C_in % GN_GROUPS) return 0;
+    if ((C_out <= 4 || C_out == 6 || C_out == 8 || C_out == 16) && (C_in == 32 || C_in == 64 || C_in == 128)) return 1;
+    return (sh + 15) / 16 * 16 + head_fold_lds(C_in) <= 64 * 1024 ? 1 : 0;
+}
+
+extern "C" int tq_head_conv_fwd_fold(const float* x, const TqGnFold* fold, float* gscale, float* gshift, const float* w,
+                                     const float* bias, const float* c_out, const float* c_skip, const float* skip_src, float* y,
+                                     int B, int T, int C_in, int C_out, int ktaps, hipStream_t stream) {
+    if (!x || !w || !y || !fold || !gscale || !gshift) return TQ_ERR_ARG;
+    if (!fold->stats0 || !fold->gamma || !fold->beta) return TQ_ERR_ARG;
+    if (c_out && (!c_skip || !skip_src)) return TQ_ERR_ARG;
+    const int slot = fold->slot0 ? fold->slot0 : STAT_SLOT;
+    if (slot != STAT_SLOT && slot != 32) return TQ_ERR_ARG;
+    if (B <= 0 || T <= 0 || !tq_head_conv_folds(C_in, C_out, ktaps)) return TQ_ERR_SHAPE;
+    HeadFold hf;
+    hf.st = fold->stats0; hf.gamma = fold->gamma; hf.beta = fold->beta;
+    hf.gscale = gscale; hf.gshift = gshift; hf.mean_rstd = fold->mean_rstd;
+    hf.nslots = (T + slot - 1) / slot; hf.lds_off = 0;
+    return head_conv_launch<true>(x, gscale, gshift, w, bias, c_out, c_skip, skip_src, y, B, T, C_in, C_out, ktaps, hf, stream);
 }
 
 namespace {
diff --git a/tqdne_amd/engine.py b/tqdne_amd/engine.py
--- a/tqdne_amd/engine.py
+++ b/tqdne_amd/engine.py
@@ -45,7 +45,8 @@
 FUSE_SKIP_CO = 32
 SMALL_TILE_B = 4
 SMALL_TILE_WGS = 64
-GN_FOLD_DEFAULT = os.environ.get("TQDNE_GN_FOLD", "0") == "1"
+GN_FOLD_DEFAULT = os.environ.get("TQDNE_GN_FOLD", "1") != "0"
+GN_FOLD_HEAD = os.environ.get("TQDNE_GN_FOLD_HEAD", "0") == "1"
 CONCURRENT_LANE0 = 8
 
 
@@ -358,6 +359,7 @@
         self.wide_stem = self.wide_head = False
         self.x_btc = self.stem_out = self.stem_rec = None
         self.final = self.head_gn = self.head_btc = self.head_rec = self.out_nct = None
+        self.head_fold = None
         self.out_mode = "head"
         self._build()
         assert self._pending_gn is None, "a deferred GroupNorm finalisation was never placed"
@@ -455,16 +457,21 @@
             out = self._act(site.C_out, T_out, stats, slot=32 if small else STAT_SLOT) if launch else None
         d = TqConvDesc()
         d.t_tile = 32 if small else 0
+        fold_flag = 0
         pend = self._pending_gn
         if pend is not None and gn is not None and pend["key"] == gn[0].data_ptr():
             self._pending_gn = None
-            fold_max = self.lib.tq_conv1d_gn_fold_max_cin(wfmt, 32 if small else 0, site.C_out)
+            fold_max = self.lib.tq_conv1d_gn_fold_max_cin_flags(wfmt, 32 if small else 0, site.C_out, _lib.TQ_CONV_FOLD_BF16X3)
             if small and wfmt != _lib.TQ_WFMT_BF16X3:
                 fold_max = min(fold_max, self.lib.tq_conv1d_gn_fold_max_cin(_lib.TQ_WFMT_BF16X3, 32, site.C_out))
             fold_fits = site.C_in <= fold_max
-            fold_default = (GN_FOLD_DEFAULT and not small and k5_act and wfmt == _lib.TQ_WFMT_F16_MX6 and self.scheme == "auto"
-                            and getattr(self.m, "_conv_scheme", "auto") == "auto" and fold_fits)
-            if fold_default and launch and not self.ckpt:
+            fold_default = (GN_FOLD_DEFAULT and not small and (k5_act or (site.K == 1 and not silu and stride == 1 and not upsample))
+                            and wfmt in (_lib.TQ_WFMT_F16_MX6, _lib.TQ_WFMT_BF16X3) and fold_fits)
+            fold_stays = wfmt == _lib.TQ_WFMT_BF16X3 or site.C_in <= self.lib.tq_conv1d_gn_fold_max_cin_flags(
+                _lib.TQ_WFMT_BF16X3, 0, site.C_out, _lib.TQ_CONV_FOLD_BF16X3)
+            if fold_default and not fold_stays and not (self.scheme == "auto" and getattr(self.m, "_conv_scheme", "auto") == "auto"):
+                fold_default = False
+            if fold_default and not fold_stays and launch and not self.ckpt:
                 fn, fargs, fname, ffl = pend["fin"][0]
                 self._fold_default_ops.append((len(self.ops), fn, d))
                 self._emit((_noop_launch, fargs, fname + " (folded into its consumer)", ffl), nbytes=0)
@@ -477,6 +484,7 @@
                 self._keep.append(f)
                 d.gn_fold = C.pointer(f)
                 self.gn_folded += 1
+                fold_flag = 0 if small else _lib.TQ_CONV_FOLD_BF16X3
             else:
                 self._emit(pend["fin"][0], nbytes=pend["fin"][1])
         d.B, d.T_in, d.T_out = self.B, T_in, T_out
@@ -497,7 +505,7 @@
             flags |= TQ_CONV_STATS
         if site.K == 1 and self._launch_bound(T_out):
             flags |= _lib.TQ_CONV_CH_TILES
-        d.flags = flags
+        d.flags = flags | fold_flag
         d.emb_stride = self.emb_total
         d.wfmt = wfmt
         if launch:
@@ -632,7 +640,17 @@
         self.wide_head = m.out[2].out_channels > NARROW_SIGNAL_CHANNELS
         if not self.wide_head:
             _check_head_limits(h.C, m.out[2].out_channels, m.out[2].kernel_size[0])
-        self.head_gn = self._gn([h], m.out[0])
+        head_folds = (GN_FOLD_DEFAULT and GN_FOLD_HEAD and not self.wide_head and not self.ckpt
+                      and bool(self.lib.tq_head_conv_folds(h.C, m.out[2].out_channels, m.out[2].kernel_size[0])))
+        self.head_gn = self._gn([h], m.out[0], defer=head_folds)
+        if head_folds:
+            pend, self._pending_gn = self._pending_gn, None
+            f = _lib.TqGnFold()
+            f.stats0, f.stats1, f.slot0, f.slot1 = _p(h.stats), None, h.slot, 0
+            f.gamma, f.beta, f.mean_rstd = _p(m.out[0].weight), _p(m.out[0].bias), _p(pend["mean_rstd"])
+            self._keep.append(f)
+            self.head_fold = f
+            self.gn_folded += 1
         if self.wide_head:
             self.out_mode = "wide"
             self._wide_head(h, m.out[2], "out.2", self.head_gn)
@@ -701,8 +719,12 @@
         e0 = _recorded_event() if trace is not None else None
         if self.out_mode == "head":
             gn = self.head_gn or (None, None)
-            check(self.lib.tq_head_conv_fwd(_p(fin.buf), _p(gn[0]), _p(gn[1]), _p(head.weight), _p(head.bias), _p(c_out), _p(c_skip),
-                                            _p(skip_src), _p(self.out_nct), B, T, fin.C, co, K, stream), what)
+            if self.head_fold is not None:
+                check(self.lib.tq_head_conv_fwd_fold(_p(fin.buf), C.byref(self.head_fold), _p(gn[0]), _p(gn[1]), _p(head.weight), _p(head.bias),
+                                                     _p(c_out), _p(c_skip), _p(skip_src), _p(self.out_nct), B, T, fin.C, co, K, stream), what)
+            else:
+                check(self.lib.tq_head_conv_fwd(_p(fin.buf), _p(gn[0]), _p(gn[1]), _p(head.weight), _p(head.bias), _p(c_out), _p(c_skip),
+                                                _p(skip_src), _p(self.out_nct), B, T, fin.C, co, K, stream), what)
             entry = (name, 2 * B * T * fin.C * co * K, 4 * B * T * (fin.C + io))
         elif self.out_mode == "wide":
             check(self.lib.tq_btc_to_nct(_p(self.head_btc.buf), _p(c_out), _p(c_skip), _p(skip_src), _p(self.out_nct), B, T,
@@ -773,7 +795,7 @@
         return out
 
     def _attention(self, x: Act, ab, name: str) -> Act:
-        g = self._gn([x], ab.norm)
+        g = self._gn([x], ab.norm, defer=not self.ckpt)
         D = ab.channels // ab.num_heads
         hd = D not in (32, 64, 128)
         if hd and not self.lib.tq_attention_head_tile(D):
diff --git a/tqdne_amd/ops.py b/tqdne_amd/ops.py
--- a/tqdne_amd/ops.py
+++ b/tqdne_amd/ops.py
@@ -31,7 +31,7 @@
 
 def conv1d(x0, weight, bias=None, *, x1=None, gscale=None, gshift=None, silu=False, emb=None, residual=None,
            stride=1, upsample=False, stats=True, dropout_p=0.0, dropout_seed=0, dropout_site=0, skip=None, wfmt=None, t_tile=0,
-           gn_fold=None, wide_table=False, out=None, pad_cout=0):
+           gn_fold=None, wide_table=False, out=None, pad_cout=0, fold_bf16x3=False):
     lib = _lib.load()
     B, T_in, C0 = x0.shape
     C1 = 0 if x1 is None else x1.shape[2]
@@ -65,6 +65,8 @@
         f |= TQ_CONV_DROPOUT
     if wide_table:
         f |= _lib.TQ_CONV_WIDE_TABLE
+    if fold_bf16x3:
+        f |= _lib.TQ_CONV_FOLD_BF16X3
     d.flags = f
     d.emb_stride = 0 if emb is None else emb.stride(0)
     d.dropout_site, d.dropout_p, d.dropout_seed = dropout_site, dropout_p, dropout_seed
```

Result: no change. 355.7, median of 6 (+0.4%).
